# xandercai/JSPSR

Hardware: AMD Instinct MI355X
Metric: Mpixels/sec fwd+bwd, JSPSR x8 on 512^2 DEM tiles (higher is better)
Workload: dtype bf16; 1 GPU; jspsr_r8_img_msk (image+mask guided, 43.87M params), 8 x 512x512 tiles per GPU, train step (fwd + L1/L2/Sobel loss + bwd + grad all-reduce + AdamW); storage policy: bf16 activations / gradients / MFMA operands, fp32 accumulation, BatchNorm statistics, master weights and optimizer, and the generator head (affinity logits + offsets) kept as fp32 planes; tiles_per_gpu=8, tile=512, global_tiles=8, parallelism=dp1, step_mode=eager

## Files before the change

### include/jspsr_hip.h

```cpp
#ifndef JSPSR_HIP_H
#define JSPSR_HIP_H

#include <stddef.h>
#include <stdint.h>

#ifdef __cplusplus
extern "C" {
#endif

#define JSPSR_OK 0
#define JSPSR_EINVAL (-1)
#define JSPSR_EALIGN (-2)

typedef void* jspsr_stream_t;

int jspsr_abi_version(void);
long long jspsr_launch_count(const char* what);
int jspsr_conv_dynamic_queue(int on);
const char* jspsr_last_error(void);

int jspsr_prop_forward_f32(const float* dem, const float* weight, const float* offset,
                           int offset_channels, const float* wk, const float* b0, float scale,
                           float* out, int B, int H, int W, jspsr_stream_t stream);

size_t jspsr_prop_backward_workspace_bytes(int B, int H, int W);

int jspsr_prop_backward_f32(const float* grad_out, const float* dem, const float* weight,
                            const float* offset, int offset_channels, const float* wk,
                            float* grad_weight, float* grad_offset, float* grad_wk,
                            float* grad_b0, void* workspace, int B, int H, int W,
                            jspsr_stream_t stream);

int jspsr_prop_backward_fold_f32(const void* workspace, int B, int H, int W, float* grad_wk, float* grad_b0,
                                 jspsr_stream_t stream);

int jspsr_prop_step_forward_f32(const float* dem, const float* weight, const float* offset, int offset_channels,
                                const float* wk, const float* b0, float scale, int normalize, float* out,
                                int B, int H, int W, jspsr_stream_t stream);
size_t jspsr_prop_step_backward_workspace_bytes(int B, int H, int W);
int jspsr_prop_step_backward_f32(const float* grad_out, const float* dem, const float* weight, const float* offset,
                                 int offset_channels, const float* wk, float scale, int normalize, int accumulate,
                                 float* grad_weight, float* grad_offset, float* grad_dem, float* grad_wk,
                                 float* grad_b0, void* workspace, int B, int H, int W, jspsr_stream_t stream);

int jspsr_prop_head_forward(int dtype, const float* dem, const void* head, const float* wk, const float* b0,
                            float scale, float* out, int B, int H, int W, jspsr_stream_t stream);
size_t jspsr_prop_head_backward_workspace_bytes(int B, int H, int W);
int jspsr_prop_head_backward(int dtype, const float* grad_out, const float* dem, const void* head, const float* wk,
                             void* grad_head, float* grad_wk, float* grad_b0, void* workspace, int B, int H, int W,
                             jspsr_stream_t stream);

int jspsr_tiles_crop_f32(const float* x, float* out, int C, int H, int W, int k, int stride, int n_x, jspsr_stream_t stream);
int jspsr_tiles_merge_f32(const float* tiles, const float* ramp, float* out, int n_x, int k, int border_px, int stride,
                          jspsr_stream_t stream);
int jspsr_mirror_pad_f32(const float* x, float* out, int C, int H, int W, int n, jspsr_stream_t stream);
int jspsr_elev_scale_f32(const float* in, float* out, long long n, int descale, int elev_log, double elev_min, double elev_max,
                         double base_elev, jspsr_stream_t stream);

#define JSPSR_BATCH_LOG 1
#define JSPSR_BATCH_SCALE_MASK 2
#define JSPSR_BATCH_IMAGE_11 4
#define JSPSR_BATCH_LABEL_11 8
#define JSPSR_BATCH_IMAGE_255 16
#define JSPSR_BATCH_FLAGS 31
int jspsr_batch_make(const void* const* src, const long long* src_bytes, float* const* out, const int* channels,
                     const int* coff, const int* cpitch, const long long* scenes, int n_scenes, const int* samples, int B,
                     int k, int flags, double elev_min, double elev_max, int mask_div, jspsr_stream_t stream);

int jspsr_prop_logits_forward_f32(const float* dem, const float* head, const float* wk, const float* b0, float scale,
                                  float* out, int B, int H, int W, jspsr_stream_t stream);
int jspsr_prop_logits_backward_f32(const float* grad_out, const float* dem, const float* head, const float* wk,
                                   float* grad_head, float* grad_wk, float* grad_b0, void* workspace, int B, int H, int W,
                                   jspsr_stream_t stream);

int jspsr_head_ok(int dtype, int B, int H, int W, int Cin);
int jspsr_head_forward(int dtype, const void* x, int x_cstride, int x_coff, int Cin, const float* w25, const float* b25,
                       float* planes, int B, int H, int W, jspsr_stream_t stream);
size_t jspsr_head_backward_workspace_bytes(int B, int H, int W);
int jspsr_head_backward(int dtype, const float* grad_planes, const float* w25, int Cin, void* grad_x, int gx_cstride,
                        int gx_coff, void* grad_nhwc32, float* grad_b25, void* workspace, int B, int H, int W,
                        jspsr_stream_t stream);

int jspsr_conv_head1_forward(int dtype, const void* x, int x_cstride, int x_coff, int C, const float* w, const float* bias,
                             float* y, int B, int H, int W, jspsr_stream_t stream);
size_t jspsr_conv_head1_workspace_bytes(int B, int H, int W, int C);
int jspsr_conv_head1_backward(int dtype, const float* dy, const void* x, int x_cstride, int x_coff, int C, const float* w,
                              void* dx, int dx_cstride, int dx_coff, float* dw, float* db, void* workspace, int B, int H,
                              int W, jspsr_stream_t stream);

#define JSPSR_F32 0
#define JSPSR_BF16 1

int jspsr_pack_weight(int dtype, const float* w, void* packed, int O, int I, int KH, int KW,
                      int mode, int c_pad, jspsr_stream_t stream);

typedef struct jspsr_pack_desc {
  const float* w;
  void* out;
  long long start;
  long long total;
  int O, I, KH, KW;
  int mode;
  int c_pad;
  int dtype;
  int reserved;
} jspsr_pack_desc;
int jspsr_pack_chunk(void);
int jspsr_pack_weights_multi(const jspsr_pack_desc* descs, int n, long long total_blocks, jspsr_stream_t stream);

int jspsr_conv2d_stats_rows(int B, int OH, int OW);
int jspsr_conv2d_in_affine_ok(int dtype, int Cin, int KH, int KW, int stride);
int jspsr_conv2d_forward(int dtype, const void* in, const void* wpack, const float* bias, void* out,
                         int B, int IH, int IW, int Cin, int in_cstride, int in_coff, int Cout,
                         int out_cstride, int out_coff, int KH, int KW, int stride, int pad, int relu,
                         float* stats, const float* scale, const void* addend, int add_cstride,
                         const float* in_affine, int in_relu, jspsr_stream_t stream);

int jspsr_conv2d_dgrad_reduce_ok(int dtype, int B, int IH, int IW, int Cg, int Cin, int KH, int KW, int stride, int pad);
int jspsr_conv2d_dgrad(int dtype, const void* gout, const void* wpack_t, const float* bias, void* gin,
                       int B, int OH, int OW, int Cg, int g_cstride, int g_coff, int IH, int IW,
                       int Cin, int in_cstride, int in_coff, int KH, int KW, int stride, int pad,
                       int relu, const void* addend, int add_cstride, const float* scale,
                       const void* red_x, int red_cstride, const float* red_par, float* red_out, jspsr_stream_t stream);

size_t jspsr_conv2d_wgrad_workspace_bytes(int dtype, int B, int OH, int OW, int Cg, int Cx, int KH, int KW);
int jspsr_conv2d_wgrad_x_affine_ok(int dtype, int B, int OH, int OW, int Cg, int Cx, int KH, int KW, int stride, int pad);
int jspsr_conv2d_wgrad(int dtype, const void* G, int Cg, int g_cstride, int g_coff, const void* X, int Cx,
                       int x_cstride, int x_coff, float* dW, int R, int C, int B, int OH, int OW,
                       int IH, int IW, int KH, int KW, int stride, int pad, int accumulate,
                       const float* x_affine, int x_relu, void* workspace, jspsr_stream_t stream);

size_t jspsr_reduce_workspace_bytes(int dtype, int C, int nseg);

int jspsr_bn_forward(int dtype, const void* x, int x_cs, int x_coff, const void* res, int r_cs, int r_coff,
                     void* y, int y_cs, int y_coff, const float* gamma, const float* beta,
                     float* running_mean, float* running_var, float momentum, float eps, int training,
                     int relu, float res_scale, float* save_mean, float* save_invstd, long long npix, int C,
                     const float* ext_partial, int ext_rows, const float* res_affine, float* affine_out,
                     void* workspace, jspsr_stream_t stream);

int jspsr_bn_fold(const float* gamma, const float* beta, const float* running_mean, const float* running_var,
                  float eps, float res_scale, int C, float* scale, float* shift, jspsr_stream_t stream);

int jspsr_bn_reduce_params(const float* gamma, const float* beta, const float* save_mean, const float* save_invstd, int C,
                           float* par, jspsr_stream_t stream);
int jspsr_bn_backward(int dtype, const void* dy, int dy_cs, int dy_coff, const void* y, int y_cs, int y_coff,
                      const void* x, int x_cs, int x_coff, const float* gamma, const float* beta, const float* save_mean,
                      const float* save_invstd, int training, int relu, float res_scale, void* dx, void* dres,
                      float* dgamma, float* dbeta, int accumulate, long long npix, int C, void* workspace,
                      const float* ext_partial, int ext_rows, jspsr_stream_t stream);

int jspsr_act_backward(int dtype, const void* dy, int dy_cs, int dy_coff, const void* y, int y_cs, int relu, void* dz,
                       int dz_cs, float* dbias, long long npix, int C, void* workspace, jspsr_stream_t stream);

int jspsr_gate_pool(int dtype, const void* x, int B, long long npix, int C, float* avg, float* mx, int* amax,
                    void* workspace, jspsr_stream_t stream);
int jspsr_gate_scale(int dtype, const void* x, const float* s, void* y, int B, long long npix, int C,
                     jspsr_stream_t stream);
int jspsr_gate_backward_reduce(int dtype, const void* dy, const void* x, float* ds, int B, long long npix, int C,
                               void* workspace, jspsr_stream_t stream);
int jspsr_gate_backward_apply(int dtype, const void* dy, const float* s, const float* davg, const float* dmax,
                              const int* amax, void* dx, int B, long long npix, int C, jspsr_stream_t stream);

size_t jspsr_loss_workspace_bytes(int B, int H, int W);
int jspsr_loss_forward(const float* pred, const float* gt, float w1, float w2, float wg, float* losses,
                       void* workspace, int B, int H, int W, jspsr_stream_t stream);
int jspsr_loss_backward(const float* pred, const float* gt, const float* grad_total, float w1, float w2,
                        float wg, float* grad_pred, const void* workspace, int B, int H, int W,
                        jspsr_stream_t stream);

size_t jspsr_loss_menu_workspace_bytes(int terms, int planes, int H, int W);
int jspsr_loss_menu_forward(const float* pred, const float* gt, int terms, int planes, int H, int W, int n_keys,
                            const int* key_slot, const double* key_weight, const float* base_losses, float* out,
                            void* workspace, jspsr_stream_t stream);
int jspsr_loss_menu_backward(const float* pred, const float* gt, int terms, int planes, int H, int W,
                             const double* slot_weight, const float* grad_total, float* grad_pred,
                             const void* workspace, jspsr_stream_t stream);
size_t jspsr_ssim_workspace_bytes(int planes, int H, int W, int same);
int jspsr_ssim_forward(const float* pred, const float* gt, int planes, int H, int W, int same, const float* window11,
                       float* out, void* workspace, jspsr_stream_t stream);

size_t jspsr_metrics_workspace_bytes(int H, int W);
int jspsr_metrics_forward(const float* pred, const float* gt, int H, int W, float border, float value_min,
                          float value_max, int elev_log, float* scores, void* workspace, jspsr_stream_t stream);

size_t jspsr_scores_batch_workspace_bytes(int B, int H, int W);
int jspsr_scores_batch_forward(const float* pred, const float* gt, int B, int H, int W, float border, float value_min,
                               float value_max, int elev_log, float* scores, void* workspace, jspsr_stream_t stream);

int jspsr_adamw_step(float* param, const float* grad, float* exp_avg, float* exp_avg_sq, long long n, float lr,
                     float beta1, float beta2, float eps, float weight_decay, int step, jspsr_stream_t stream);
int jspsr_adamw_step_dev(float* param, const float* grad, float* exp_avg, float* exp_avg_sq, long long n,
                         const float* hyper, jspsr_stream_t stream);

#define JSPSR_OPT_SGD 0
#define JSPSR_OPT_ADAM 1
#define JSPSR_OPT_ADAMW 2
#define JSPSR_OPT_RMSPROP 3
size_t jspsr_optim_workspace_bytes(void);
int jspsr_optim_step(int kind, float* param, const float* grad, float* state1, float* state2, long long n, float lr, float a,
                     float b, float eps, float weight_decay, int step, const float* hyper, float* grad_range, void* workspace,
                     jspsr_stream_t stream);
size_t jspsr_tensor_ranges_workspace_bytes(void);
int jspsr_tensor_ranges(int count, const void* const* tensors, const long long* numel, const int* dtypes, float* table,
                        void* workspace, jspsr_stream_t stream);

int jspsr_gate_mlp_forward(const float* avg, const float* mx, const float* w1, const float* w2, int B, int C, int Ch,
                           float* s, float* hid, jspsr_stream_t stream);
size_t jspsr_gate_mlp_backward_workspace_bytes(int B, int C, int Ch);
int jspsr_gate_mlp_backward(const float* ds, const float* s, const float* hid, const float* avg, const float* mx,
                            const float* w1, const float* w2, int B, int C, int Ch, float* davg, float* dmax, float* dw1,
                            float* dw2, void* workspace, jspsr_stream_t stream);

int jspsr_nchw_to_nhwc(int dtype, const float* src, void* dst, int B, int C, int H, int W, int c_pad, jspsr_stream_t stream);

#ifdef __cplusplus
}
#endif
#endif
```

### jspsr_amd/_lib.py

```python
from __future__ import annotations

import ctypes
import os
import subprocess
import threading

_HERE = os.path.dirname(os.path.abspath(__file__))
SO_PATH = os.environ.get("JSPSR_LAB_LIB") or os.path.join(_HERE, "lib", "libjspsr_hip.so")
CSRC = os.path.join(_HERE, "csrc")
ABI_VERSION = 20

_lock = threading.Lock()
_lib = None

c_p = ctypes.c_void_p
c_i = ctypes.c_int
c_f = ctypes.c_float
c_ll = ctypes.c_longlong

SIGNATURES = {
    "jspsr_abi_version": (c_i, []),
    "jspsr_launch_count": (c_ll, [ctypes.c_char_p]),
    "jspsr_conv_dynamic_queue": (c_i, [c_i]),
    "jspsr_last_error": (ctypes.c_char_p, []),
    "jspsr_prop_forward_f32": (c_i, [c_p, c_p, c_p, c_i, c_p, c_p, c_f, c_p, c_i, c_i, c_i, c_p]),
    "jspsr_prop_backward_workspace_bytes": (ctypes.c_size_t, [c_i, c_i, c_i]),
    "jspsr_prop_backward_f32": (c_i, [c_p] * 4 + [c_i] + [c_p] * 6 + [c_i, c_i, c_i, c_p]),
    "jspsr_prop_backward_fold_f32": (c_i, [c_p, c_i, c_i, c_i, c_p, c_p, c_p]),
    "jspsr_prop_step_forward_f32": (c_i, [c_p, c_p, c_p, c_i, c_p, c_p, c_f, c_i, c_p, c_i, c_i, c_i, c_p]),
    "jspsr_prop_step_backward_workspace_bytes": (ctypes.c_size_t, [c_i, c_i, c_i]),
    "jspsr_prop_step_backward_f32": (c_i, [c_p] * 4 + [c_i, c_p, c_f, c_i, c_i] + [c_p] * 6 + [c_i, c_i, c_i, c_p]),
    "jspsr_prop_head_forward": (c_i, [c_i, c_p, c_p, c_p, c_p, c_f, c_p, c_i, c_i, c_i, c_p]),
    "jspsr_prop_head_backward_workspace_bytes": (ctypes.c_size_t, [c_i, c_i, c_i]),
    "jspsr_prop_head_backward": (c_i, [c_i] + [c_p] * 8 + [c_i, c_i, c_i, c_p]),
    "jspsr_prop_logits_forward_f32": (c_i, [c_p, c_p, c_p, c_p, c_f, c_p, c_i, c_i, c_i, c_p]),
    "jspsr_prop_logits_backward_f32": (c_i, [c_p] * 8 + [c_i, c_i, c_i, c_p]),
    "jspsr_head_ok": (c_i, [c_i] * 5),
    "jspsr_head_forward": (c_i, [c_i, c_p, c_i, c_i, c_i, c_p, c_p, c_p, c_i, c_i, c_i, c_p]),
    "jspsr_head_backward_workspace_bytes": (ctypes.c_size_t, [c_i, c_i, c_i]),
    "jspsr_head_backward": (c_i, [c_i, c_p, c_p, c_i, c_p, c_i, c_i, c_p, c_p, c_p, c_i, c_i, c_i, c_p]),
    "jspsr_conv_head1_forward": (c_i, [c_i, c_p, c_i, c_i, c_i, c_p, c_p, c_p, c_i, c_i, c_i, c_p]),
    "jspsr_conv_head1_workspace_bytes": (ctypes.c_size_t, [c_i, c_i, c_i, c_i]),
    "jspsr_conv_head1_backward": (c_i, [c_i, c_p, c_p, c_i, c_i, c_i, c_p, c_p, c_i, c_i, c_p, c_p, c_p, c_i, c_i, c_i, c_p]),
    "jspsr_pack_weight": (c_i, [c_i, c_p, c_p] + [c_i] * 6 + [c_p]),
    "jspsr_pack_chunk": (c_i, []),
    "jspsr_pack_weights_multi": (c_i, [c_p, c_i, c_ll, c_p]),
    "jspsr_conv2d_stats_rows": (c_i, [c_i, c_i, c_i]),
    "jspsr_conv2d_in_affine_ok": (c_i, [c_i] * 5),
    "jspsr_conv2d_forward": (c_i, [c_i] + [c_p] * 4 + [c_i] * 14 + [c_p, c_p, c_p, c_i, c_p, c_i, c_p]),
    "jspsr_bn_fold": (c_i, [c_p, c_p, c_p, c_p, c_f, c_f, c_i, c_p, c_p, c_p]),
    "jspsr_conv2d_dgrad_reduce_ok": (c_i, [c_i] * 10),
    "jspsr_conv2d_dgrad": (c_i, [c_i] + [c_p] * 4 + [c_i] * 16 + [c_p, c_i, c_p, c_p, c_i, c_p, c_p, c_p]),
    "jspsr_conv2d_wgrad_workspace_bytes": (ctypes.c_size_t, [c_i] * 8),
    "jspsr_conv2d_wgrad_x_affine_ok": (c_i, [c_i] * 10),
    "jspsr_conv2d_wgrad": (c_i, [c_i, c_p, c_i, c_i, c_i, c_p, c_i, c_i, c_i, c_p] + [c_i] * 12 + [c_p, c_i, c_p, c_p]),
    "jspsr_reduce_workspace_bytes": (ctypes.c_size_t, [c_i, c_i, c_i]),
    "jspsr_bn_forward": (c_i, [c_i, c_p, c_i, c_i, c_p, c_i, c_i, c_p, c_i, c_i, c_p, c_p, c_p, c_p, c_f, c_f, c_i,
                               c_i, c_f, c_p, c_p, c_ll, c_i, c_p, c_i, c_p, c_p, c_p, c_p]),
    "jspsr_bn_reduce_params": (c_i, [c_p, c_p, c_p, c_p, c_i, c_p, c_p]),
    "jspsr_bn_backward": (c_i, [c_i, c_p, c_i, c_i, c_p, c_i, c_i, c_p, c_i, c_i, c_p, c_p, c_p, c_p, c_i, c_i, c_f,
                                c_p, c_p, c_p, c_p, c_i, c_ll, c_i, c_p, c_p, c_i, c_p]),
    "jspsr_act_backward": (c_i, [c_i, c_p, c_i, c_i, c_p, c_i, c_i, c_p, c_i, c_p, c_ll, c_i, c_p, c_p]),
    "jspsr_gate_pool": (c_i, [c_i, c_p, c_i, c_ll, c_i, c_p, c_p, c_p, c_p, c_p]),
    "jspsr_gate_scale": (c_i, [c_i, c_p, c_p, c_p, c_i, c_ll, c_i, c_p]),
    "jspsr_gate_backward_reduce": (c_i, [c_i, c_p, c_p, c_p, c_i, c_ll, c_i, c_p, c_p]),
    "jspsr_gate_backward_apply": (c_i, [c_i, c_p, c_p, c_p, c_p, c_p, c_p, c_i, c_ll, c_i, c_p]),
    "jspsr_loss_workspace_bytes": (ctypes.c_size_t, [c_i, c_i, c_i]),
    "jspsr_loss_forward": (c_i, [c_p, c_p, c_f, c_f, c_f, c_p, c_p, c_i, c_i, c_i, c_p]),
    "jspsr_loss_backward": (c_i, [c_p, c_p, c_p, c_f, c_f, c_f, c_p, c_p, c_i, c_i, c_i, c_p]),
    "jspsr_loss_menu_workspace_bytes": (ctypes.c_size_t, [c_i, c_i, c_i, c_i]),
    "jspsr_loss_menu_forward": (c_i, [c_p, c_p, c_i, c_i, c_i, c_i, c_i, c_p, c_p, c_p, c_p, c_p, c_p]),
    "jspsr_loss_menu_backward": (c_i, [c_p, c_p, c_i, c_i, c_i, c_i, c_p, c_p, c_p, c_p, c_p]),
    "jspsr_ssim_workspace_bytes": (ctypes.c_size_t, [c_i, c_i, c_i, c_i]),
    "jspsr_ssim_forward": (c_i, [c_p, c_p, c_i, c_i, c_i, c_i, c_p, c_p, c_p, c_p]),
    "jspsr_metrics_workspace_bytes": (ctypes.c_size_t, [c_i, c_i]),
    "jspsr_metrics_forward": (c_i, [c_p, c_p, c_i, c_i, c_f, c_f, c_f, c_i, c_p, c_p, c_p]),
    "jspsr_scores_batch_workspace_bytes": (ctypes.c_size_t, [c_i, c_i, c_i]),
    "jspsr_scores_batch_forward": (c_i, [c_p, c_p, c_i, c_i, c_i, c_f, c_f, c_f, c_i, c_p, c_p, c_p]),
    "jspsr_adamw_step": (c_i, [c_p, c_p, c_p, c_p, c_ll, c_f, c_f, c_f, c_f, c_f, c_i, c_p]),
    "jspsr_adamw_step_dev": (c_i, [c_p, c_p, c_p, c_p, c_ll, c_p, c_p]),
    "jspsr_optim_workspace_bytes": (ctypes.c_size_t, []),
    "jspsr_optim_step": (c_i, [c_i, c_p, c_p, c_p, c_p, c_ll, c_f, c_f, c_f, c_f, c_f, c_i, c_p, c_p, c_p, c_p]),
    "jspsr_tensor_ranges_workspace_bytes": (ctypes.c_size_t, []),
    "jspsr_tensor_ranges": (c_i, [c_i, c_p, c_p, c_p, c_p, c_p, c_p]),
    "jspsr_tiles_crop_f32":(c_i, [c_p, c_p] + [c_i] * 6 + [c_p]),
    "jspsr_tiles_merge_f32": (c_i, [c_p, c_p, c_p, c_i, c_i, c_i, c_i, c_p]),
    "jspsr_mirror_pad_f32": (c_i, [c_p, c_p, c_i, c_i, c_i, c_i, c_p]),
    "jspsr_elev_scale_f32": (c_i, [c_p, c_p, c_ll, c_i, c_i, ctypes.c_double, ctypes.c_double, ctypes.c_double, c_p]),
    "jspsr_gate_mlp_forward": (c_i, [c_p, c_p, c_p, c_p, c_i, c_i, c_i, c_p, c_p, c_p]),
    "jspsr_gate_mlp_backward_workspace_bytes": (ctypes.c_size_t, [c_i, c_i, c_i]),
    "jspsr_gate_mlp_backward": (c_i, [c_p] * 7 + [c_i, c_i, c_i] + [c_p] * 6),
    "jspsr_batch_make": (c_i, [c_p] * 7 + [c_i, c_p, c_i, c_i, c_i, ctypes.c_double, ctypes.c_double, c_i, c_p]),
    "jspsr_nchw_to_nhwc": (c_i, [c_i, c_p, c_p, c_i, c_i, c_i, c_i, c_i, c_p]),
}


class JspsrHipError(RuntimeError):
    pass


def build(verbose: bool = False) -> str:
    cmd = ["make", "-C", CSRC, "-j4"] + ([] if verbose else ["-s"])
    subprocess.check_call(cmd)
    return SO_PATH


def load():
    global _lib
    if _lib is not None:
        return _lib
    with _lock:
        if _lib is not None:
            return _lib
        if not os.path.exists(SO_PATH):
            raise JspsrHipError(
                f"{SO_PATH} is missing: build it with `python -c 'import __graft_entry__ as g; g.build()'` "
                "(hipcc --offload-arch=gfx950). jspsr_amd has no fallback path."
            )
        import torch
        lib = ctypes.CDLL(SO_PATH)
        for name, (res, args) in SIGNATURES.items():
            fn = getattr(lib, name)
            fn.restype = res
            fn.argtypes = args
        v = lib.jspsr_abi_version()
        if v != ABI_VERSION:
            raise JspsrHipError(f"libjspsr_hip.so ABI {v} != binding ABI {ABI_VERSION}: rebuild")
        _lib = lib
    return _lib


calls = 0


def check(code: int, what: str):
    global calls
    calls += 1
    if code != 0:
        msg = load().jspsr_last_error().decode(errors="replace")
        raise JspsrHipError(f"{what} failed (code {code}): {msg}")
```

### jspsr_amd/csrc/common.hip

```cpp
#include "common.h"

#include <atomic>
#include <cstring>

namespace jspsr {

namespace {
struct Slot {
  std::atomic<const char*> name{nullptr};
  std::atomic<long long> n{0};
};
Slot g_slots[128];

void count_launch(const char* what) {
  for (Slot& s : g_slots) {
    const char* cur = s.name.load(std::memory_order_acquire);
    if (cur == nullptr) {
      const char* expect = nullptr;
      if (s.name.compare_exchange_strong(expect, what, std::memory_order_acq_rel)) cur = what; else cur = expect;
    }
    if (cur == what) { s.n.fetch_add(1, std::memory_order_relaxed); return; }
  }
}
}

char* err_buf() {
  static thread_local char buf[512] = {0};
  return buf;
}

int fail(int code, const char* fmt, ...) {
  va_list ap;
  va_start(ap, fmt);
  vsnprintf(err_buf(), 512, fmt, ap);
  va_end(ap);
  return code;
}

int check_launch(const char* what) {
  count_launch(what);
  hipError_t e = hipGetLastError();
  if (e != hipSuccess) return fail(static_cast<int>(e), "%s: %s", what, hipGetErrorString(e));
  return JSPSR_OK;
}

}

namespace jspsr {
std::atomic<int> g_conv_dynq{-1};
int conv_dynq_override() { return g_conv_dynq.load(std::memory_order_relaxed); }
}

extern "C" int jspsr_abi_version(void) { return 20; }
extern "C" int jspsr_conv_dynamic_queue(int on) { return jspsr::g_conv_dynq.exchange(on < 0 ? -1 : (on ? 1 : 0), std::memory_order_relaxed); }
extern "C" long long jspsr_launch_count(const char* what) {
  if (!what) return -1;
  long long n = 0;
  for (jspsr::Slot& s : jspsr::g_slots) {
    const char* cur = s.name.load(std::memory_order_acquire);
    if (cur && strcmp(cur, what) == 0) n += s.n.load(std::memory_order_relaxed);
  }
  return n;
}
extern "C" const char* jspsr_last_error(void) { return jspsr::err_buf(); }
```

### jspsr_amd/csrc/elementwise.hip

```cpp
#include "common.h"

#include <cstdlib>

namespace {

using namespace jspsr;

constexpr int TX = 64, TY = 4;

template <typename T> struct V;
template <> struct V<float> { static constexpr int N = 4; };
template <> struct V<__bf16> { static constexpr int N = 8; };

template <typename T, int N>
struct Pack { T v[N]; };

template <typename T>
__device__ __forceinline__ uint4 load_raw(const T* p) { return *reinterpret_cast<const uint4*>(p); }
template <typename T>
__device__ __forceinline__ void unpack(const uint4& raw, float (&f)[V<T>::N]) {
  if constexpr (sizeof(T) == 4) {
    f[0] = __uint_as_float(raw.x); f[1] = __uint_as_float(raw.y); f[2] = __uint_as_float(raw.z); f[3] = __uint_as_float(raw.w);
  } else {
    const unsigned w[4] = {raw.x, raw.y, raw.z, raw.w};
#pragma unroll
    for (int i = 0; i < 4; ++i) {
      f[2 * i] = __uint_as_float(w[i] << 16);
      f[2 * i + 1] = __uint_as_float(w[i] & 0xffff0000u);
    }
  }
}

__device__ __forceinline__ unsigned bf16_bits(float x) {
  const __bf16 h = (__bf16)x;
  return (unsigned)__builtin_bit_cast(unsigned short, h);
}

template <typename T>
__device__ __forceinline__ void store_vec(T* p, const float (&f)[V<T>::N]) {
  uint4 raw;
  if constexpr (sizeof(T) == 4) {
    raw.x = __float_as_uint(f[0]); raw.y = __float_as_uint(f[1]); raw.z = __float_as_uint(f[2]); raw.w = __float_as_uint(f[3]);
  } else {
    raw.x = bf16_bits(f[0]) | (bf16_bits(f[1]) << 16);
    raw.y = bf16_bits(f[2]) | (bf16_bits(f[3]) << 16);
    raw.z = bf16_bits(f[4]) | (bf16_bits(f[5]) << 16);
    raw.w = bf16_bits(f[6]) | (bf16_bits(f[7]) << 16);
  }
  *reinterpret_cast<uint4*>(p) = raw;
}

struct Slice {
  const void* p;
  int cs, coff;
};

struct RedGeom {
  long long npix;
  int nseg;
  int C;
  int chunks;
  long long chunk_pix;
  int lpp;
  int pl;
};

struct LaneMap {
  int c;
  int sub;
};
template <int N>
__device__ __forceinline__ LaneMap lane_map(const RedGeom& g) {
  LaneMap m;
  const int tx = threadIdx.x;
  m.sub = tx / g.lpp;
  const int cg = blockIdx.y * TX + (tx - m.sub * g.lpp);
  m.c = (m.sub < g.pl) ? cg * N : g.C;
  return m;
}

RedGeom make_red(long long npix, int nseg, int C, int vec) {
  RedGeom g;
  g.npix = npix; g.nseg = nseg; g.C = C;
  const int gy = (C / vec + TX - 1) / TX;
  static const int target = [] { const char* e = getenv("JSPSR_RED_BLOCKS"); return e ? atoi(e) : 1024; }();
  long long want = target / ((long long)gy * nseg);
  if (want < 1) want = 1;
  long long chunks = (npix + 63) / 64;
  if (chunks > want) chunks = want;
  if (chunks < 1) chunks = 1;
  g.chunk_pix = (npix + chunks - 1) / chunks;
  g.chunks = (int)((npix + g.chunk_pix - 1) / g.chunk_pix);
  const int groups = C / vec;
  g.lpp = groups < TX ? groups : TX;
  g.pl = TX / g.lpp;
  return g;
}
dim3 red_grid(const RedGeom& g, int vec) { return dim3(g.nseg * g.chunks, (g.C / vec + TX - 1) / TX); }

#ifndef K4_PIX_FLY
#define K4_PIX_FLY 4
#endif
constexpr int PIX_FLY = K4_PIX_FLY;
template <typename T, int K, int NTEN, typename L, typename F>
__device__ __forceinline__ void reduce_pixels_mlp(const RedGeom& g, float* __restrict__ partial, L&& load, F&& use) {
  constexpr int N = V<T>::N;
  __shared__ float red[TY][K][TX * N];
  const int tx = threadIdx.x, ty = threadIdx.y;
  const LaneMap lm = lane_map<N>(g);
  const int c = lm.c;
  const int seg = blockIdx.x / g.chunks, chunk = blockIdx.x % g.chunks;
  float acc[K][N];
#pragma unroll
  for (int k = 0; k < K; ++k)
#pragma unroll
    for (int i = 0; i < N; ++i) acc[k][i] = 0.f;
  const long long p0 = chunk * g.chunk_pix;
  const long long p1 = (p0 + g.chunk_pix < g.npix) ? p0 + g.chunk_pix : g.npix;
  if (c < g.C) {
    const long long step = TY * g.pl, base = (long long)seg * g.npix;
    long long p = p0 + ty * g.pl + lm.sub;
    for (; p + (PIX_FLY - 1) * step < p1; p += PIX_FLY * step) {
      uint4 raw[PIX_FLY][NTEN];
#pragma unroll
      for (int u = 0; u < PIX_FLY; ++u) load(base + p + u * step, c, raw[u]);
#pragma unroll
      for (int u = 0; u < PIX_FLY; ++u) use(base + p + u * step, c, raw[u], acc);
    }
    for (; p < p1; p += step) {
      uint4 raw[NTEN];
      load(base + p, c, raw);
      use(base + p, c, raw, acc);
    }
  }
#pragma unroll
  for (int k = 0; k < K; ++k)
#pragma unroll
    for (int i = 0; i < N; ++i) red[ty][k][tx * N + i] = acc[k][i];
  __syncthreads();
  if (ty == 0 && lm.sub == 0 && c < g.C) {
    float* dst = partial + ((size_t)blockIdx.x * K) * g.C + c;
#pragma unroll
    for (int k = 0; k < K; ++k)
#pragma unroll
      for (int i = 0; i < N; ++i) {
        float s = 0.f;
        for (int j = 0; j < g.pl; ++j)
#pragma unroll
          for (int y = 0; y < TY; ++y) s += red[y][k][(tx + j * g.lpp) * N + i];
        dst[(size_t)k * g.C + i] = s;
      }
  }
}
template <typename T, int NTEN, typename L, typename F>
__device__ __forceinline__ void for_pixels_mlp(const RedGeom& g, L&& load, F&& use) {
  constexpr int N = V<T>::N;
  const LaneMap lm = lane_map<N>(g);
  const int c = lm.c;
  if (c >= g.C) return;
  const int seg = blockIdx.x / g.chunks, chunk = blockIdx.x % g.chunks;
  const long long p0 = chunk * g.chunk_pix;
  const long long p1 = (p0 + g.chunk_pix < g.npix) ? p0 + g.chunk_pix : g.npix;
  const long long step = TY * g.pl, base = (long long)seg * g.npix;
  long long p = p0 + threadIdx.y * g.pl + lm.sub;
  for (; p + (PIX_FLY - 1) * step < p1; p += PIX_FLY * step) {
    uint4 raw[PIX_FLY][NTEN];
#pragma unroll
    for (int u = 0; u < PIX_FLY; ++u) load(base + p + u * step, c, raw[u]);
#pragma unroll
    for (int u = 0; u < PIX_FLY; ++u) use(p + u * step, base + p + u * step, c, raw[u]);
  }
  for (; p < p1; p += step) {
    uint4 raw[NTEN];
    load(base + p, c, raw);
    use(p, base + p, c, raw);
  }
}

template <int N>
__device__ __forceinline__ void load_param(const float* __restrict__ p, float (&f)[N]) {
#pragma unroll
  for (int i = 0; i < N; i += 4) {
    const float4 v = *reinterpret_cast<const float4*>(p + i);
    f[i] = v.x; f[i + 1] = v.y; f[i + 2] = v.z; f[i + 3] = v.w;
  }
}

__device__ __forceinline__ double wave_sum_rows(const float* __restrict__ partial, int rows, size_t pitch, size_t off) {
  const int lane = threadIdx.x & 63;
  double s = 0.0;
  for (int r = lane; r < rows; r += 64) s += (double)partial[(size_t)r * pitch + off];
#pragma unroll
  for (int d = 32; d > 0; d >>= 1) s += __shfl_xor(s, d, 64);
  return s;
}

__device__ __forceinline__ void wave_sum_rows2(const float* __restrict__ partial, int rows, size_t pitch, size_t off0, size_t off1,
                                               double& s0, double& s1) {
  const int lane = threadIdx.x & 63;
  double a = 0.0, b = 0.0;
  int r = lane;
  for (; r + 192 < rows; r += 256) {
    const float x0 = partial[(size_t)r * pitch + off0], x1 = partial[(size_t)(r + 64) * pitch + off0];
    const float x2 = partial[(size_t)(r + 128) * pitch + off0], x3 = partial[(size_t)(r + 192) * pitch + off0];
    const float y0 = partial[(size_t)r * pitch + off1], y1 = partial[(size_t)(r + 64) * pitch + off1];
    const float y2 = partial[(size_t)(r + 128) * pitch + off1], y3 = partial[(size_t)(r + 192) * pitch + off1];
    a += (double)x0; a += (double)x1; a += (double)x2; a += (double)x3;
    b += (double)y0; b += (double)y1; b += (double)y2; b += (double)y3;
  }
  for (; r < rows; r += 64) {
    a += (double)partial[(size_t)r * pitch + off0];
    b += (double)partial[(size_t)r * pitch + off1];
  }
#pragma unroll
  for (int d = 32; d > 0; d >>= 1) {
    a += __shfl_xor(a, d, 64);
    b += __shfl_xor(b, d, 64);
  }
  s0 = a;
  s1 = b;
}

template <typename T>
__global__ __launch_bounds__(TX * TY) void bn_stats_kernel(const T* __restrict__ x, int cs, int coff, RedGeom g,
                                                          float* __restrict__ partial) {
  constexpr int N = V<T>::N;
  reduce_pixels_mlp<T, 2, 1>(
      g, partial, [&](long long pix, int c, uint4 (&raw)[1]) { raw[0] = load_raw<T>(x + (size_t)pix * cs + coff + c); },
      [&](long long, int, const uint4 (&raw)[1], float (&acc)[2][N]) {
        float f[N];
        unpack<T>(raw[0], f);
#pragma unroll
        for (int i = 0; i < N; ++i) { acc[0][i] += f[i]; acc[1][i] += f[i] * f[i]; }
      });
}

__global__ void fold_rows_kernel(const float* __restrict__ in, int nin, int width, int nout, float* __restrict__ out) {
  const int r = blockIdx.x, j = blockIdx.y * blockDim.x + threadIdx.x;
  if (j >= width) return;
  float s = 0.f;
  int i = r;
  for (; i + 7 * nout < nin; i += 8 * nout) {
    float v[8];
#pragma unroll
    for (int k = 0; k < 8; ++k) v[k] = in[(size_t)(i + k * nout) * width + j];
#pragma unroll
    for (int k = 0; k < 8; ++k) s += v[k];
  }
  for (; i < nin; i += nout) s += in[(size_t)i * width + j];
  out[(size_t)r * width + j] = s;
}

__global__ void bn_finalize_kernel(const float* __restrict__ partial, int rows, int C, long long count,
                                   const float* __restrict__ gamma, const float* __restrict__ beta,
                                   float* __restrict__ running_mean, float* __restrict__ running_var,
                                   float momentum, float eps, int training, float* __restrict__ save_mean,
                                   float* __restrict__ save_invstd, float* __restrict__ scale,
                                   float* __restrict__ shift) {
  const int c = blockIdx.x * (blockDim.x >> 6) + (threadIdx.x >> 6);
  if (c >= C) return;
  float mean, var;
  double s = 0.0, ss = 0.0;
  if (training) {
    wave_sum_rows2(partial, rows, (size_t)2 * C, c, (size_t)C + c, s, ss);
  }
  if ((threadIdx.x & 63) != 0) return;
  if (training) {
    const double m = s / (double)count;
    double v = ss / (double)count - m * m;
    if (v < 0.0) v = 0.0;
    mean = (float)m;
    var = (float)v;
    if (running_mean) {
      const double unb = count > 1 ? v * (double)count / (double)(count - 1) : v;
      running_mean[c] = (1.f - momentum) * running_mean[c] + momentum * mean;
      running_var[c] = (1.f - momentum) * running_var[c] + momentum * (float)unb;
    }
  } else {
    mean = running_mean[c];
    var = running_var[c];
  }
  const float invstd = 1.0f / sqrtf(var + eps);
  save_mean[c] = mean;
  save_invstd[c] = invstd;
  const float sc = gamma[c] * invstd;
  scale[c] = sc;
  shift[c] = beta[c] - mean * sc;
}

__global__ void bn_fold_kernel(const float* __restrict__ gamma, const float* __restrict__ beta,
                               const float* __restrict__ mean, const float* __restrict__ var, float eps, float res_scale,
                               int C, float* __restrict__ scale, float* __restrict__ shift) {
  const int c = blockIdx.x * blockDim.x + threadIdx.x;
  if (c >= C) return;
  const float sc = gamma[c] * (1.0f / sqrtf(var[c] + eps));
  scale[c] = sc * res_scale;
  shift[c] = (beta[c] - mean[c] * sc) * res_scale;
}

template <typename T, bool RES>
__global__ __launch_bounds__(TX * TY) void bn_apply_kernel(const T* __restrict__ x, int x_cs, int x_coff,
                                                          const T* __restrict__ res, int r_cs, int r_coff,
                                                          T* __restrict__ y, int y_cs, int y_coff,
                                                          const float* __restrict__ scale, const float* __restrict__ shift,
                                                          const float* __restrict__ raff, float res_scale, int relu, RedGeom g) {
  constexpr int N = V<T>::N;
  float sc[N], sh[N], rsc[N], rsh[N];
  const int c0 = lane_map<N>(g).c;
  if (c0 < g.C) { load_param<N>(scale + c0, sc); load_param<N>(shift + c0, sh); }
  if (raff && c0 < g.C) { load_param<N>(raff + c0, rsc); load_param<N>(raff + g.C + c0, rsh); }
  constexpr int NTEN = RES ? 2 : 1;
  for_pixels_mlp<T, NTEN>(
      g,
      [&](long long pix, int c, uint4 (&raw)[NTEN]) {
        raw[0] = load_raw<T>(x + (size_t)pix * x_cs + x_coff + c);
        if constexpr (RES) raw[1] = load_raw<T>(res + (size_t)pix * r_cs + r_coff + c);
      },
      [&](long long, long long pix, int c, const uint4 (&raw)[NTEN]) {
        float f[N], r[N];
        unpack<T>(raw[0], f);
        if constexpr (RES) unpack<T>(raw[1], r);
#pragma unroll
        for (int k = 0; k < N; ++k) {
          float v = f[k] * sc[k] + sh[k];
          if (RES) v = v * res_scale + (raff ? r[k] * rsc[k] + rsh[k] : r[k]);
          if (relu) v = fmaxf(v, 0.f);
          f[k] = v;
        }
        store_vec<T>(y + (size_t)pix * y_cs + y_coff + c, f);
      });
}

template <typename T, int RELU>
__global__ __launch_bounds__(TX * TY) void bn_bwd_reduce_kernel(const T* __restrict__ dy, int dy_cs, int dy_coff,
                                                               const T* __restrict__ y, int y_cs, int y_coff,
                                                               const T* __restrict__ x, int x_cs, int x_coff,
                                                               const float* __restrict__ mean,
                                                               const float* __restrict__ invstd,
                                                               const float* __restrict__ gamma,
                                                               const float* __restrict__ beta, RedGeom g,
                                                               float* __restrict__ partial) {
  constexpr int N = V<T>::N, NTEN = RELU == 1 ? 3 : 2;
  float mu[N], is[N], ga[N], be[N];
  const int c0 = lane_map<N>(g).c;
  if (c0 < g.C) {
    load_param<N>(mean + c0, mu); load_param<N>(invstd + c0, is);
    if (RELU == 2) { load_param<N>(gamma + c0, ga); load_param<N>(beta + c0, be); }
  }
  reduce_pixels_mlp<T, 2, NTEN>(
      g, partial,
      [&](long long pix, int c, uint4 (&raw)[NTEN]) {
        raw[0] = load_raw<T>(dy + (size_t)pix * dy_cs + dy_coff + c);
        raw[1] = load_raw<T>(x + (size_t)pix * x_cs + x_coff + c);
        if constexpr (RELU == 1) raw[2] = load_raw<T>(y + (size_t)pix * y_cs + y_coff + c);
      },
      [&](long long, int, const uint4 (&raw)[NTEN], float (&acc)[2][N]) {
        float d[N], xv[N], yv[N];
        unpack<T>(raw[0], d);
        unpack<T>(raw[1], xv);
        if constexpr (RELU == 1) unpack<T>(raw[2], yv);
#pragma unroll
        for (int i = 0; i < N; ++i) {
          const float xhat = (xv[i] - mu[i]) * is[i];
          const bool off = RELU == 1 ? !(yv[i] > 0.f) : (RELU == 2 ? !(ga[i] * xhat + be[i] > 0.f) : false);
          const float dz = off ? 0.f : d[i];
          acc[0][i] += dz;
          acc[1][i] += dz * xhat;
        }
      });
}

__global__ void bn_bwd_finalize_kernel(const float* __restrict__ partial, int rows, int C, long long count,
                                       const float* __restrict__ gamma, const float* __restrict__ invstd,
                                       int training, float res_scale, int accumulate, float* __restrict__ dgamma,
                                       float* __restrict__ dbeta, float* __restrict__ coef) {
  const int c = blockIdx.x * (blockDim.x >> 6) + (threadIdx.x >> 6);
  if (c >= C) return;
  double s, sx;
  wave_sum_rows2(partial, rows, (size_t)2 * C, c, (size_t)C + c, s, sx);
  if ((threadIdx.x & 63) != 0) return;
  dbeta[c] = (accumulate ? dbeta[c] : 0.f) + (float)(s * res_scale);
  dgamma[c] = (accumulate ? dgamma[c] : 0.f) + (float)(sx * res_scale);
  const float k = gamma[c] * invstd[c] * res_scale;
  coef[c] = k;
  coef[C + c] = training ? (float)(s / (double)count) : 0.f;
  coef[2 * C + c] = training ? (float)(sx / (double)count) : 0.f;
}

template <typename T, int RELU>
__global__ __launch_bounds__(TX * TY) void bn_bwd_apply_kernel(const T* __restrict__ dy, int dy_cs, int dy_coff,
                                                              const T* __restrict__ y, int y_cs, int y_coff,
                                                              const T* __restrict__ x, int x_cs, int x_coff,
                                                              const float* __restrict__ mean, const float* __restrict__ invstd,
                                                              const float* __restrict__ gamma, const float* __restrict__ beta,
                                                              const float* __restrict__ coef,
                                                              T* __restrict__ dx, T* __restrict__ dres, RedGeom g) {
  constexpr int N = V<T>::N, NTEN = RELU == 1 ? 3 : 2;
  const int C = g.C;
  float mu[N], is[N], k0[N], ka[N], kb[N], ga[N], be[N];
  const int c0 = lane_map<N>(g).c;
  if (c0 < C) {
    load_param<N>(mean + c0, mu); load_param<N>(invstd + c0, is);
    load_param<N>(coef + c0, k0); load_param<N>(coef + C + c0, ka); load_param<N>(coef + 2 * C + c0, kb);
    if (RELU == 2) { load_param<N>(gamma + c0, ga); load_param<N>(beta + c0, be); }
  }
  for_pixels_mlp<T, NTEN>(
      g,
      [&](long long pix, int c, uint4 (&raw)[NTEN]) {
        raw[0] = load_raw<T>(dy + (size_t)pix * dy_cs + dy_coff + c);
        raw[1] = load_raw<T>(x + (size_t)pix * x_cs + x_coff + c);
        if constexpr (RELU == 1) raw[2] = load_raw<T>(y + (size_t)pix * y_cs + y_coff + c);
      },
      [&](long long, long long pix, int c, const uint4 (&raw)[NTEN]) {
        float d[N], xv[N], yv[N], o[N];
        unpack<T>(raw[0], d);
        unpack<T>(raw[1], xv);
        if constexpr (RELU == 1) unpack<T>(raw[2], yv);
#pragma unroll
        for (int k = 0; k < N; ++k) {
          const float xhat = (xv[k] - mu[k]) * is[k];
          const bool off = RELU == 1 ? !(yv[k] > 0.f) : (RELU == 2 ? !(ga[k] * xhat + be[k] > 0.f) : false);
          const float dz = off ? 0.f : d[k];
          d[k] = dz;
          o[k] = k0[k] * (dz - ka[k] - xhat * kb[k]);
        }
        store_vec<T>(dx + (size_t)pix * C + c, o);
        if (dres) store_vec<T>(dres + (size_t)pix * C + c, d);
      });
}

template <typename T, bool RELU>
__global__ __launch_bounds__(TX * TY) void act_bwd_kernel(const T* __restrict__ dy, int dy_cs, int dy_coff,
                                                         const T* __restrict__ y, int y_cs, int relu,
                                                         T* __restrict__ dz, int dz_cs, RedGeom g,
                                                         float* __restrict__ partial) {
  constexpr int N = V<T>::N;
  constexpr int NTEN = RELU ? 2 : 1;
  (void)relu;
  reduce_pixels_mlp<T, 1, NTEN>(
      g, partial,
      [&](long long pix, int c, uint4 (&raw)[NTEN]) {
        raw[0] = load_raw<T>(dy + (size_t)pix * dy_cs + dy_coff + c);
        if constexpr (RELU) raw[1] = load_raw<T>(y + (size_t)pix * y_cs + c);
      },
      [&](long long pix, int c, const uint4 (&raw)[NTEN], float (&acc)[1][N]) {
        float d[N], yv[N];
        unpack<T>(raw[0], d);
        if constexpr (RELU) unpack<T>(raw[1], yv);
#pragma unroll
        for (int i = 0; i < N; ++i) {
          if (RELU && !(yv[i] > 0.f)) d[i] = 0.f;
          acc[0][i] += d[i];
        }
        if (dz) store_vec<T>(dz + (size_t)pix * dz_cs + c, d);
      });
}

__global__ void sum_rows_kernel(const float* __restrict__ partial, int rows, int K, int k, int C, float* __restrict__ out) {
  const int c = blockIdx.x * (blockDim.x >> 6) + (threadIdx.x >> 6);
  if (c >= C) return;
  const double s = wave_sum_rows(partial, rows, (size_t)K * C, (size_t)k * C + c);
  if ((threadIdx.x & 63) == 0) out[c] = (float)s;
}

template <typename T>
__global__ __launch_bounds__(TX * TY) void gate_pool_kernel(const T* __restrict__ x, RedGeom g,
                                                           float* __restrict__ psum, float* __restrict__ pmax,
                                                           int* __restrict__ pidx) {
  constexpr int N = V<T>::N;
  __shared__ float rs[TY][TX * N], rm[TY][TX * N];
  __shared__ int ri[TY][TX * N];
  const int tx = threadIdx.x, ty = threadIdx.y;
  const LaneMap lm = lane_map<N>(g);
  const int c = lm.c;
  const int seg = blockIdx.x / g.chunks, chunk = blockIdx.x % g.chunks;
  float s[N], m[N];
  int idx[N];
#pragma unroll
  for (int i = 0; i < N; ++i) { s[i] = 0.f; m[i] = -INFINITY; idx[i] = 0x7fffffff; }
  const long long p0 = chunk * g.chunk_pix;
  const long long p1 = (p0 + g.chunk_pix < g.npix) ? p0 + g.chunk_pix : g.npix;
  if (c < g.C) {
    const long long step = TY * g.pl;
    long long p = p0 + ty * g.pl + lm.sub;
    auto take = [&](const uint4& raw, long long pp) {
      float f[N];
      unpack<T>(raw, f);
#pragma unroll
      for (int i = 0; i < N; ++i) {
        s[i] += f[i];
        if (f[i] > m[i]) { m[i] = f[i]; idx[i] = (int)pp; }
      }
    };
    for (; p + (PIX_FLY - 1) * step < p1; p += PIX_FLY * step) {
      uint4 raw[PIX_FLY];
#pragma unroll
      for (int u = 0; u < PIX_FLY; ++u) raw[u] = load_raw<T>(x + ((size_t)seg * g.npix + p + u * step) * g.C + c);
#pragma unroll
      for (int u = 0; u < PIX_FLY; ++u) take(raw[u], p + u * step);
    }
    for (; p < p1; p += step) take(load_raw<T>(x + ((size_t)seg * g.npix + p) * g.C + c), p);
  }
#pragma unroll
  for (int i = 0; i < N; ++i) { rs[ty][tx * N + i] = s[i]; rm[ty][tx * N + i] = m[i]; ri[ty][tx * N + i] = idx[i]; }
  __syncthreads();
  if (ty == 0 && lm.sub == 0 && c < g.C) {
#pragma unroll
    for (int i = 0; i < N; ++i) {
      float ss = 0.f, mm = -INFINITY;
      int ii = 0x7fffffff;
      for (int q = 0; q < g.pl; ++q)
#pragma unroll
      for (int y = 0; y < TY; ++y) {
        const int col = (tx + q * g.lpp) * N + i;
        ss += rs[y][col];
        const float v = rm[y][col];
        const int j = ri[y][col];
        if (v > mm || (v == mm && j < ii)) { mm = v; ii = j; }
      }
      const size_t o = (size_t)blockIdx.x * g.C + c + i;
      psum[o] = ss; pmax[o] = mm; pidx[o] = ii;
    }
  }
}

__global__ void gate_pool_finalize_kernel(const float* __restrict__ psum, const float* __restrict__ pmax,
                                          const int* __restrict__ pidx, int chunks, int C, long long npix,
                                          float* __restrict__ avg, float* __restrict__ mx, int* __restrict__ amax) {
  const int c = blockIdx.x * blockDim.x + threadIdx.x, b = blockIdx.y;
  if (c >= C) return;
  double s = 0.0;
  float m = -INFINITY;
  int ii = 0x7fffffff;
  int r = 0;
  for (; r + 8 <= chunks; r += 8) {
    float ps[8], pm[8];
    int pi[8];
#pragma unroll
    for (int k = 0; k < 8; ++k) {
      const size_t o = ((size_t)b * chunks + r + k) * C + c;
      ps[k] = psum[o]; pm[k] = pmax[o]; pi[k] = pidx[o];
    }
#pragma unroll
    for (int k = 0; k < 8; ++k) {
      s += (double)ps[k];
      if (pm[k] > m || (pm[k] == m && pi[k] < ii)) { m = pm[k]; ii = pi[k]; }
    }
  }
  for (; r < chunks; ++r) {
    const size_t o = ((size_t)b * chunks + r) * C + c;
    s += (double)psum[o];
    if (pmax[o] > m || (pmax[o] == m && pidx[o] < ii)) { m = pmax[o]; ii = pidx[o]; }
  }
  avg[(size_t)b * C + c] = (float)(s / (double)npix);
  mx[(size_t)b * C + c] = m;
  amax[(size_t)b * C + c] = ii;
}

template <typename T>
__global__ __launch_bounds__(TX * TY) void gate_scale_kernel(const T* __restrict__ x, const float* __restrict__ s,
                                                            T* __restrict__ y, RedGeom g) {
  constexpr int N = V<T>::N;
  float sv[N];
  const int c0 = lane_map<N>(g).c;
  if (c0 < g.C) load_param<N>(s + (size_t)(blockIdx.x / g.chunks) * g.C + c0, sv);
  for_pixels_mlp<T, 1>(
      g, [&](long long pix, int c, uint4 (&raw)[1]) { raw[0] = load_raw<T>(x + (size_t)pix * g.C + c); },
      [&](long long, long long pix, int c, const uint4 (&raw)[1]) {
        float f[N];
        unpack<T>(raw[0], f);
#pragma unroll
        for (int k = 0; k < N; ++k) f[k] *= sv[k];
        store_vec<T>(y + (size_t)pix * g.C + c, f);
      });
}

template <typename T>
__global__ __launch_bounds__(TX * TY) void gate_bwd_reduce_kernel(const T* __restrict__ dy, const T* __restrict__ x,
                                                                 RedGeom g, float* __restrict__ partial) {
  constexpr int N = V<T>::N;
  reduce_pixels_mlp<T, 1, 2>(
      g, partial,
      [&](long long pix, int c, uint4 (&raw)[2]) {
        raw[0] = load_raw<T>(dy + (size_t)pix * g.C + c);
        raw[1] = load_raw<T>(x + (size_t)pix * g.C + c);
      },
      [&](long long, int, const uint4 (&raw)[2], float (&acc)[1][N]) {
        float d[N], xv[N];
        unpack<T>(raw[0], d);
        unpack<T>(raw[1], xv);
#pragma unroll
        for (int i = 0; i < N; ++i) acc[0][i] += d[i] * xv[i];
      });
}

__global__ void gate_bwd_finalize_kernel(const float* __restrict__ partial, int chunks, int C, float* __restrict__ ds) {
  const int c = blockIdx.x * blockDim.x + threadIdx.x, b = blockIdx.y;
  if (c >= C) return;
  double s = 0.0;
  int r = 0;
  for (; r + 8 <= chunks; r += 8) {
    float v[8];
#pragma unroll
    for (int k = 0; k < 8; ++k) v[k] = partial[((size_t)b * chunks + r + k) * C + c];
#pragma unroll
    for (int k = 0; k < 8; ++k) s += (double)v[k];
  }
  for (; r < chunks; ++r) s += (double)partial[((size_t)b * chunks + r) * C + c];
  ds[(size_t)b * C + c] = (float)s;
}

template <typename T>
__global__ __launch_bounds__(TX * TY) void gate_bwd_apply_kernel(const T* __restrict__ dy, const float* __restrict__ s,
                                                                const float* __restrict__ davg, const float* __restrict__ dmax,
                                                                const int* __restrict__ amax, T* __restrict__ dx, RedGeom g) {
  constexpr int N = V<T>::N;
  float sv[N], da[N], dm[N];
  int am[N];
  const int c0 = lane_map<N>(g).c;
  const float inv = 1.f / (float)g.npix;
  if (c0 < g.C) {
    const size_t o = (size_t)(blockIdx.x / g.chunks) * g.C + c0;
    load_param<N>(s + o, sv); load_param<N>(davg + o, da); load_param<N>(dmax + o, dm);
#pragma unroll
    for (int k = 0; k < N; ++k) { am[k] = amax[o + k]; da[k] *= inv; }
  }
  for_pixels_mlp<T, 1>(
      g, [&](long long pix, int c, uint4 (&raw)[1]) { raw[0] = load_raw<T>(dy + (size_t)pix * g.C + c); },
      [&](long long p, long long pix, int c, const uint4 (&raw)[1]) {
        float f[N];
        unpack<T>(raw[0], f);
#pragma unroll
        for (int k = 0; k < N; ++k) f[k] = f[k] * sv[k] + da[k] + (am[k] == (int)p ? dm[k] : 0.f);
        store_vec<T>(dx + (size_t)pix * g.C + c, f);
      });
}

int ew_blocks(long long total) {
  long long b = (total + 255) / 256;
  return (int)(b < 1 ? 1 : (b > 4096 ? 4096 : b));
}

int check_c(int dtype, int C, const char* what) {
  if (dtype != JSPSR_F32 && dtype != JSPSR_BF16) return fail(JSPSR_EINVAL, "%s: bad dtype", what);
  const int vec = dtype == JSPSR_F32 ? 4 : 8;
  if (C <= 0 || C % vec) return fail(JSPSR_EINVAL, "%s: C=%d must be a multiple of %d", what, C, vec);
  return JSPSR_OK;
}

}

#define DISPATCH(dtype, CALL)                    \
  do {                                           \
    if ((dtype) == JSPSR_F32) { using T = float; CALL; } else { using T = __bf16; CALL; } \
  } while (0)

extern "C" size_t jspsr_reduce_workspace_bytes(int dtype, int C, int nseg) {
  if (C <= 0 || nseg <= 0) return 0;
  const int vec = dtype == JSPSR_F32 ? 4 : 8;
  const RedGeom g = make_red(1LL << 40, nseg, C, vec);
  const size_t rows = (size_t)nseg * g.chunks;
  return (rows * 3 + 4) * (size_t)C * sizeof(float) + 64;
}

extern "C" int jspsr_bn_forward(int dtype, const void* x, int x_cs, int x_coff, const void* res, int r_cs, int r_coff,
                                void* y, int y_cs, int y_coff, const float* gamma, const float* beta,
                                float* running_mean, float* running_var, float momentum, float eps, int training,
                                int relu, float res_scale, float* save_mean, float* save_invstd, long long npix, int C,
                                const float* ext_partial, int ext_rows, const float* res_affine, float* affine_out,
                                void* workspace, jspsr_stream_t stream) {
  if (int e = check_c(dtype, C, "bn_forward")) return e;
  if (!x || (!y && !affine_out) || !gamma || !beta || !save_mean || !save_invstd || !workspace || npix <= 0)
    return fail(JSPSR_EINVAL, "bn_forward: null pointer or empty tensor");
  if (res_affine && !res) return fail(JSPSR_EINVAL, "bn_forward: res_affine without a residual operand");
  if (!training && (!running_mean || !running_var)) return fail(JSPSR_EINVAL, "bn_forward: eval mode needs running stats");
  const int vec = dtype == JSPSR_F32 ? 4 : 8;
  if (x_cs % vec || x_coff % vec || y_cs % vec || y_coff % vec || (res && (r_cs % vec || r_coff % vec)))
    return fail(JSPSR_EINVAL, "bn_forward: channel pitches/offsets must be multiples of %d", vec);
  hipStream_t s = static_cast<hipStream_t>(stream);
  float* ws = static_cast<float*>(workspace);
  float* scale = affine_out ? affine_out : ws;
  float* shift = affine_out ? affine_out + C : ws + C;
  float* partial = ws + 2 * C;
  int rows = 0;
  if (training && ext_partial) {
    if (ext_rows <= 0) return fail(JSPSR_EINVAL, "bn_forward: ext_rows must be positive");
    rows = ext_rows < 256 ? ext_rows : 256;
    if (ext_rows > 256) {
      hipLaunchKernelGGL(fold_rows_kernel, dim3(rows, (2 * C + 255) / 256), dim3(256), 0, s, ext_partial, ext_rows, 2 * C, rows, partial);
      if (int e = check_launch("bn_fold_rows")) return e;
    } else {
      (void)hipMemcpyAsync(partial, ext_partial, (size_t)ext_rows * 2 * C * sizeof(float), hipMemcpyDeviceToDevice, s);
    }
  } else if (training) {
    const RedGeom g = make_red(npix, 1, C, vec);
    rows = g.chunks;
    DISPATCH(dtype, hipLaunchKernelGGL(bn_stats_kernel<T>, red_grid(g, vec), dim3(TX, TY), 0, s,
                                       static_cast<const T*>(x), x_cs, x_coff, g, partial));
    if (int e = check_launch("bn_stats")) return e;
  }
  hipLaunchKernelGGL(bn_finalize_kernel, dim3((C + 3) / 4), dim3(256), 0, s, partial, rows, C, npix, gamma, beta,
                     running_mean, running_var, momentum, eps, training, save_mean, save_invstd, scale, shift);
  if (int e = check_launch("bn_finalize")) return e;
  if (!y) return JSPSR_OK;
  const RedGeom ga = make_red(npix, 1, C, vec);
#define BN_APPLY(R) DISPATCH(dtype, hipLaunchKernelGGL((bn_apply_kernel<T, R>), red_grid(ga, vec), dim3(TX, TY), 0, s,             \
                                     static_cast<const T*>(x), x_cs, x_coff, static_cast<const T*>(res), r_cs, r_coff,        \
                                     static_cast<T*>(y), y_cs, y_coff, scale, shift, res_affine, res_scale, relu, ga))
  if (res) { BN_APPLY(true); } else { BN_APPLY(false); }
#undef BN_APPLY
  return check_launch("bn_apply");
}

__global__ void bn_reduce_params_kernel(const float* __restrict__ gamma, const float* __restrict__ beta, const float* __restrict__ mean,
                                        const float* __restrict__ invstd, int C, float* __restrict__ par) {
  const int c = blockIdx.x * blockDim.x + threadIdx.x;
  if (c >= C) return;
  const float a = gamma[c] * invstd[c];
  par[c] = a;
  par[C + c] = beta[c] - a * mean[c];
  par[2 * C + c] = invstd[c];
  par[3 * C + c] = -mean[c] * invstd[c];
}

extern "C" int jspsr_bn_reduce_params(const float* gamma, const float* beta, const float* save_mean, const float* save_invstd, int C,
                                      float* par, jspsr_stream_t stream) {
  if (!gamma || !beta || !save_mean || !save_invstd || !par || C <= 0) return fail(JSPSR_EINVAL, "bn_reduce_params: bad arguments");
  hipLaunchKernelGGL(bn_reduce_params_kernel, dim3((C + 255) / 256), dim3(256), 0, static_cast<hipStream_t>(stream), gamma, beta,
                     save_mean, save_invstd, C, par);
  return check_launch("bn_reduce_params");
}

extern "C" int jspsr_bn_backward(int dtype, const void* dy, int dy_cs, int dy_coff, const void* y, int y_cs, int y_coff,
                                 const void* x, int x_cs, int x_coff, const float* gamma, const float* beta, const float* save_mean,
                                 const float* save_invstd, int training, int relu, float res_scale, void* dx, void* dres,
                                 float* dgamma, float* dbeta, int accumulate, long long npix, int C, void* workspace,
                                 const float* ext_partial, int ext_rows, jspsr_stream_t stream) {
  if (int e = check_c(dtype, C, "bn_backward")) return e;
  if (!dy || !x || !gamma || !save_mean || !save_invstd || !dx || !dgamma || !dbeta || !workspace || npix <= 0 ||
      (relu == 1 && !y) || (relu == 2 && !beta) || relu < 0 || relu > 2)
    return fail(JSPSR_EINVAL, "bn_backward: null pointer, empty tensor or bad relu mode");
  const int vec = dtype == JSPSR_F32 ? 4 : 8;
  if (dy_cs % vec || dy_coff % vec || x_cs % vec || x_coff % vec || (relu == 1 && (y_cs % vec || y_coff % vec)))
    return fail(JSPSR_EINVAL, "bn_backward: channel pitches/offsets must be multiples of %d", vec);
  hipStream_t s = static_cast<hipStream_t>(stream);
  float* ws = static_cast<float*>(workspace);
  float* coef = ws;
  float* partial = ws + 3 * C;
  const RedGeom g = make_red(npix, 1, C, vec);
#define BN_BWD_REDUCE(R) DISPATCH(dtype, hipLaunchKernelGGL((bn_bwd_reduce_kernel<T, R>), red_grid(g, vec), dim3(TX, TY), 0, s, \
                                     static_cast<const T*>(dy), dy_cs, dy_coff, static_cast<const T*>(y), y_cs, y_coff,     \
                                     static_cast<const T*>(x), x_cs, x_coff, save_mean, save_invstd, gamma, beta, g, partial))
  int rows = g.chunks;
  if (ext_partial) {
    if (ext_rows <= 0) return fail(JSPSR_EINVAL, "bn_backward: ext_rows must be positive");
    if (ext_rows > 1024) {
      rows = g.chunks < 1024 ? (g.chunks > 0 ? g.chunks : 1) : 1024;
      hipLaunchKernelGGL(fold_rows_kernel, dim3(rows, (2 * C + 255) / 256), dim3(256), 0, s, ext_partial, ext_rows, 2 * C, rows, partial);
      if (int e = check_launch("bn_fold_rows")) return e;
    } else {
      partial = const_cast<float*>(ext_partial);
      rows = ext_rows;
    }
  } else {
    if (relu == 0) { BN_BWD_REDUCE(0); } else if (relu == 1) { BN_BWD_REDUCE(1); } else { BN_BWD_REDUCE(2); }
    if (int e = check_launch("bn_bwd_reduce")) return e;
  }
#undef BN_BWD_REDUCE
  hipLaunchKernelGGL(bn_bwd_finalize_kernel, dim3((C + 3) / 4), dim3(256), 0, s, partial, rows, C, npix, gamma,
                     save_invstd, training, res_scale, accumulate, dgamma, dbeta, coef);
  if (int e = check_launch("bn_bwd_finalize")) return e;
#define BN_BWD_APPLY(R) DISPATCH(dtype, hipLaunchKernelGGL((bn_bwd_apply_kernel<T, R>), red_grid(g, vec), dim3(TX, TY), 0, s,  \
                                     static_cast<const T*>(dy), dy_cs, dy_coff, static_cast<const T*>(y), y_cs, y_coff,     \
                                     static_cast<const T*>(x), x_cs, x_coff, save_mean, save_invstd, gamma, beta, coef,     \
                                     static_cast<T*>(dx), static_cast<T*>(dres), g))
  if (relu == 0) { BN_BWD_APPLY(0); } else if (relu == 1) { BN_BWD_APPLY(1); } else { BN_BWD_APPLY(2); }
#undef BN_BWD_APPLY
  return check_launch("bn_bwd_apply");
}

extern "C" int jspsr_bn_fold(const float* gamma, const float* beta, const float* running_mean, const float* running_var,
                             float eps, float res_scale, int C, float* scale, float* shift, jspsr_stream_t stream) {
  if (!gamma || !beta || !running_mean || !running_var || !scale || !shift || C <= 0)
    return fail(JSPSR_EINVAL, "bn_fold: bad arguments");
  hipLaunchKernelGGL(bn_fold_kernel, dim3((C + 255) / 256), dim3(256), 0, static_cast<hipStream_t>(stream), gamma, beta,
                     running_mean, running_var, eps, res_scale, C, scale, shift);
  return check_launch("bn_fold");
}

extern "C" int jspsr_act_backward(int dtype, const void* dy, int dy_cs, int dy_coff, const void* y, int y_cs, int relu,
                                  void* dz, int dz_cs, float* dbias, long long npix, int C, void* workspace,
                                  jspsr_stream_t stream) {
  if (int e = check_c(dtype, C, "act_backward")) return e;
  if (!dy || (relu && !y) || !workspace || npix <= 0) return fail(JSPSR_EINVAL, "act_backward: null pointer or empty tensor");
  const int vec = dtype == JSPSR_F32 ? 4 : 8;
  if (dy_cs % vec || dy_coff % vec || (dz && dz_cs % vec) || (relu && (y_cs % vec || y_cs < C)))
    return fail(JSPSR_EINVAL, "act_backward: bad pitch");
  hipStream_t s = static_cast<hipStream_t>(stream);
  float* partial = static_cast<float*>(workspace);
  const RedGeom g = make_red(npix, 1, C, vec);
#define ACT_BWD(R) DISPATCH(dtype, hipLaunchKernelGGL((act_bwd_kernel<T, R>), red_grid(g, vec), dim3(TX, TY), 0, s, static_cast<const T*>(dy), \
                                     dy_cs, dy_coff, static_cast<const T*>(y), y_cs, relu, static_cast<T*>(dz), dz_cs, g, partial))
  if (relu) { ACT_BWD(true); } else { ACT_BWD(false); }
#undef ACT_BWD
  if (int e = check_launch("act_backward")) return e;
  if (dbias) {
    hipLaunchKernelGGL(sum_rows_kernel, dim3((C + 3) / 4), dim3(256), 0, s, partial, g.chunks, 1, 0, C, dbias);
    return check_launch("act_backward_bias");
  }
  return JSPSR_OK;
}

extern "C" int jspsr_gate_pool(int dtype, const void* x, int B, long long npix, int C, float* avg, float* mx, int* amax,
                               void* workspace, jspsr_stream_t stream) {
  if (int e = check_c(dtype, C, "gate_pool")) return e;
  if (!x || !avg || !mx || !amax || !workspace || B <= 0 || npix <= 0 || npix > 0x7fffffffLL)
    return fail(JSPSR_EINVAL, "gate_pool: bad arguments");
  const int vec = dtype == JSPSR_F32 ? 4 : 8;
  hipStream_t s = static_cast<hipStream_t>(stream);
  const RedGeom g = make_red(npix, B, C, vec);
  const size_t rows = (size_t)B * g.chunks;
  float* psum = static_cast<float*>(workspace);
  float* pmax = psum + rows * C;
  int* pidx = reinterpret_cast<int*>(pmax + rows * C);
  DISPATCH(dtype, hipLaunchKernelGGL(gate_pool_kernel<T>, red_grid(g, vec), dim3(TX, TY), 0, s, static_cast<const T*>(x), g,
                                     psum, pmax, pidx));
  if (int e = check_launch("gate_pool")) return e;
  hipLaunchKernelGGL(gate_pool_finalize_kernel, dim3((C + 255) / 256, B), dim3(256), 0, s, psum, pmax, pidx, g.chunks, C,
                     npix, avg, mx, amax);
  return check_launch("gate_pool_finalize");
}

extern "C" int jspsr_gate_scale(int dtype, const void* x, const float* s_, void* y, int B, long long npix, int C,
                                jspsr_stream_t stream) {
  if (int e = check_c(dtype, C, "gate_scale")) return e;
  if (!x || !s_ || !y || B <= 0 || npix <= 0) return fail(JSPSR_EINVAL, "gate_scale: bad arguments");
  const int vec = dtype == JSPSR_F32 ? 4 : 8;
  hipStream_t s = static_cast<hipStream_t>(stream);
  const RedGeom g = make_red(npix, B, C, vec);
  DISPATCH(dtype, hipLaunchKernelGGL(gate_scale_kernel<T>, red_grid(g, vec), dim3(TX, TY), 0, s,
                                     static_cast<const T*>(x), s_, static_cast<T*>(y), g));
  return check_launch("gate_scale");
}

extern "C" int jspsr_gate_backward_reduce(int dtype, const void* dy, const void* x, float* ds, int B, long long npix, int C,
                                          void* workspace, jspsr_stream_t stream) {
  if (int e = check_c(dtype, C, "gate_backward_reduce")) return e;
  if (!dy || !x || !ds || !workspace || B <= 0 || npix <= 0) return fail(JSPSR_EINVAL, "gate_backward_reduce: bad arguments");
  const int vec = dtype == JSPSR_F32 ? 4 : 8;
  hipStream_t s = static_cast<hipStream_t>(stream);
  const RedGeom g = make_red(npix, B, C, vec);
  float* partial = static_cast<float*>(workspace);
  DISPATCH(dtype, hipLaunchKernelGGL(gate_bwd_reduce_kernel<T>, red_grid(g, vec), dim3(TX, TY), 0, s,
                                     static_cast<const T*>(dy), static_cast<const T*>(x), g, partial));
  if (int e = check_launch("gate_backward_reduce")) return e;
  hipLaunchKernelGGL(gate_bwd_finalize_kernel, dim3((C + 255) / 256, B), dim3(256), 0, s, partial, g.chunks, C, ds);
  return check_launch("gate_backward_finalize");
}

extern "C" int jspsr_gate_backward_apply(int dtype, const void* dy, const float* s_, const float* davg, const float* dmax,
                                         const int* amax, void* dx, int B, long long npix, int C, jspsr_stream_t stream) {
  if (int e = check_c(dtype, C, "gate_backward_apply")) return e;
  if (!dy || !s_ || !davg || !dmax || !amax || !dx || B <= 0 || npix <= 0)
    return fail(JSPSR_EINVAL, "gate_backward_apply: bad arguments");
  const int vec = dtype == JSPSR_F32 ? 4 : 8;
  hipStream_t s = static_cast<hipStream_t>(stream);
  const RedGeom g = make_red(npix, B, C, vec);
  DISPATCH(dtype, hipLaunchKernelGGL(gate_bwd_apply_kernel<T>, red_grid(g, vec), dim3(TX, TY), 0, s,
                                     static_cast<const T*>(dy), s_, davg, dmax, amax, static_cast<T*>(dx), g));
  return check_launch("gate_backward_apply");
}

template <typename T>
__global__ __launch_bounds__(256) void nchw_to_nhwc_kernel(const float* __restrict__ src, T* __restrict__ dst, int C, long long HW,
                                                          long long npix, int Cpad) {
  constexpr int N = V<T>::N;
  for (long long p = blockIdx.x * 256LL + threadIdx.x; p < npix; p += (long long)gridDim.x * 256) {
    const long long b = p / HW, q = p - b * HW;
    const float* s = src + (size_t)b * C * HW + q;
    T* d = dst + (size_t)p * Cpad;
    for (int c0 = 0; c0 < Cpad; c0 += N) {
      float f[N];
#pragma unroll
      for (int i = 0; i < N; ++i) f[i] = c0 + i < C ? s[(size_t)(c0 + i) * HW] : 0.f;
      store_vec<T>(d + c0, f);
    }
  }
}

extern "C" int jspsr_nchw_to_nhwc(int dtype, const float* src, void* dst, int B, int C, int H, int W, int c_pad,
                                  jspsr_stream_t stream) {
  if (dtype != JSPSR_F32 && dtype != JSPSR_BF16) return fail(JSPSR_EINVAL, "nchw_to_nhwc: dtype must be JSPSR_F32 or JSPSR_BF16");
  const int vec = dtype == JSPSR_F32 ? 4 : 8;
  if (!src || !dst || B <= 0 || C <= 0 || H <= 0 || W <= 0 || c_pad < C || c_pad % vec)
    return fail(JSPSR_EINVAL, "nchw_to_nhwc: bad arguments (c_pad must be a multiple of %d and >= C)", vec);
  if (!aligned4(src) || !aligned16(dst)) return fail(JSPSR_EALIGN, "nchw_to_nhwc: src must be 4-byte, dst 16-byte aligned");
  const long long HW = (long long)H * W, npix = HW * B;
  const long long want = (npix + 255) / 256;
  const int blocks = (int)(want > 8192 ? 8192 : want);
  hipStream_t s = static_cast<hipStream_t>(stream);
  DISPATCH(dtype, hipLaunchKernelGGL(nchw_to_nhwc_kernel<T>, dim3(blocks), dim3(256), 0, s, src, static_cast<T*>(dst), C, HW, npix, c_pad));
  return check_launch("nchw_to_nhwc");
}

constexpr int GM_T = 256;

__global__ __launch_bounds__(GM_T) void gate_mlp_fwd_kernel(const float* __restrict__ avg, const float* __restrict__ mx,
                                                           const float* __restrict__ w1, const float* __restrict__ w2, int C, int Ch,
                                                           float* __restrict__ s, float* __restrict__ hid) {
  extern __shared__ float gm_lds[];
  const int b = blockIdx.x, tid = threadIdx.x, wave = tid >> 6, lane = tid & 63;
  const float* a = avg + (size_t)b * C;
  const float* m = mx + (size_t)b * C;
  for (int j = wave; j < Ch; j += GM_T / 64) {
    const float* w = w1 + (size_t)j * C;
    float da = 0.f, dm = 0.f;
    for (int c = lane; c < C; c += 64) { const float wv = w[c]; da += wv * a[c]; dm += wv * m[c]; }
#pragma unroll
    for (int d = 32; d > 0; d >>= 1) { da += __shfl_xor(da, d, 64); dm += __shfl_xor(dm, d, 64); }
    if (lane == 0) {
      const float ha = fmaxf(da, 0.f), hm = fmaxf(dm, 0.f);
      hid[((size_t)b * 2 + 0) * Ch + j] = ha;
      hid[((size_t)b * 2 + 1) * Ch + j] = hm;
      gm_lds[j] = ha + hm;
    }
  }
  __syncthreads();
  for (int c = tid; c < C; c += GM_T) {
    const float* w = w2 + (size_t)c * Ch;
    float z = 0.f;
    for (int j = 0; j < Ch; ++j) z += w[j] * gm_lds[j];
    s[(size_t)b * C + c] = 1.f / (1.f + expf(-z));
  }
}

__global__ __launch_bounds__(GM_T) void gate_mlp_bwd_kernel(const float* __restrict__ ds, const float* __restrict__ s,
                                                           const float* __restrict__ hid, const float* __restrict__ w1,
                                                           const float* __restrict__ w2, int C, int Ch, float* __restrict__ davg,
                                                           float* __restrict__ dmax, float* __restrict__ dzs, float* __restrict__ dhs) {
  extern __shared__ float gm_lds[];
  float* dz = gm_lds;
  float* dh = gm_lds + C;
  const int b = blockIdx.x, tid = threadIdx.x, wave = tid >> 6, lane = tid & 63;
  for (int c = tid; c < C; c += GM_T) {
    const float sv = s[(size_t)b * C + c], v = ds[(size_t)b * C + c] * sv * (1.f - sv);
    dz[c] = v;
    dzs[(size_t)b * C + c] = v;
  }
  __syncthreads();
  for (int j = wave; j < Ch; j += GM_T / 64) {
    float acc = 0.f;
    for (int c = lane; c < C; c += 64) acc += w2[(size_t)c * Ch + j] * dz[c];
#pragma unroll
    for (int d = 32; d > 0; d >>= 1) acc += __shfl_xor(acc, d, 64);
    if (lane == 0) {
      const float da = hid[((size_t)b * 2 + 0) * Ch + j] > 0.f ? acc : 0.f, dm = hid[((size_t)b * 2 + 1) * Ch + j] > 0.f ? acc : 0.f;
      dh[j] = da; dh[Ch + j] = dm;
      dhs[((size_t)b * 2 + 0) * Ch + j] = da;
      dhs[((size_t)b * 2 + 1) * Ch + j] = dm;
    }
  }
  __syncthreads();
  for (int c = tid; c < C; c += GM_T) {
    float ga = 0.f, gm = 0.f;
    for (int j = 0; j < Ch; ++j) { const float wv = w1[(size_t)j * C + c]; ga += wv * dh[j]; gm += wv * dh[Ch + j]; }
    davg[(size_t)b * C + c] = ga;
    dmax[(size_t)b * C + c] = gm;
  }
}

__global__ __launch_bounds__(GM_T) void gate_mlp_wgrad_kernel(const float* __restrict__ dzs, const float* __restrict__ dhs,
                                                             const float* __restrict__ hid, const float* __restrict__ avg,
                                                             const float* __restrict__ mx, int B, int C, int Ch,
                                                             float* __restrict__ dw1, float* __restrict__ dw2) {
  const long long n = (long long)C * Ch;
  for (long long i = blockIdx.x * (long long)GM_T + threadIdx.x; i < 2 * n; i += (long long)gridDim.x * GM_T) {
    if (i < n) {
      const int j = (int)(i / C), c = (int)(i - (long long)j * C);
      float g = 0.f;
      for (int b = 0; b < B; ++b)
        g += dhs[((size_t)b * 2 + 0) * Ch + j] * avg[(size_t)b * C + c] + dhs[((size_t)b * 2 + 1) * Ch + j] * mx[(size_t)b * C + c];
      dw1[i] = g;
    } else {
      const long long k = i - n;
      const int c = (int)(k / Ch), j = (int)(k - (long long)c * Ch);
      float g = 0.f;
      for (int b = 0; b < B; ++b) g += dzs[(size_t)b * C + c] * (hid[((size_t)b * 2 + 0) * Ch + j] + hid[((size_t)b * 2 + 1) * Ch + j]);
      dw2[k] = g;
    }
  }
}

extern "C" int jspsr_gate_mlp_forward(const float* avg, const float* mx, const float* w1, const float* w2, int B, int C, int Ch,
                                      float* s, float* hid, jspsr_stream_t stream) {
  if (!avg || !mx || !w1 || !w2 || !s || !hid || B <= 0 || C <= 0 || Ch <= 0 || Ch > 4096)
    return fail(JSPSR_EINVAL, "gate_mlp_forward: bad arguments");
  hipLaunchKernelGGL(gate_mlp_fwd_kernel, dim3(B), dim3(GM_T), Ch * sizeof(float), static_cast<hipStream_t>(stream), avg, mx, w1, w2,
                     C, Ch, s, hid);
  return check_launch("gate_mlp_forward");
}

extern "C" size_t jspsr_gate_mlp_backward_workspace_bytes(int B, int C, int Ch) {
  if (B <= 0 || C <= 0 || Ch <= 0) return 0;
  return ((size_t)B * C + (size_t)B * 2 * Ch) * sizeof(float);
}

extern "C" int jspsr_gate_mlp_backward(const float* ds, const float* s, const float* hid, const float* avg, const float* mx,
                                       const float* w1, const float* w2, int B, int C, int Ch, float* davg, float* dmax,
                                       float* dw1, float* dw2, void* workspace, jspsr_stream_t stream) {
  if (!ds || !s || !hid || !avg || !mx || !w1 || !w2 || !davg || !dmax || !dw1 || !dw2 || !workspace || B <= 0 || C <= 0 ||
      Ch <= 0 || (size_t)(C + 2 * Ch) * sizeof(float) > 64 * 1024)
    return fail(JSPSR_EINVAL, "gate_mlp_backward: bad arguments");
  float* dzs = static_cast<float*>(workspace);
  float* dhs = dzs + (size_t)B * C;
  hipStream_t st = static_cast<hipStream_t>(stream);
  hipLaunchKernelGGL(gate_mlp_bwd_kernel, dim3(B), dim3(GM_T), (C + 2 * Ch) * sizeof(float), st, ds, s, hid, w1, w2, C, Ch, davg, dmax,
                     dzs, dhs);
  if (int e = check_launch("gate_mlp_backward")) return e;
  const long long n2 = 2LL * C * Ch;
  const int blocks = (int)((n2 + GM_T - 1) / GM_T > 2048 ? 2048 : (n2 + GM_T - 1) / GM_T);
  hipLaunchKernelGGL(gate_mlp_wgrad_kernel, dim3(blocks), dim3(GM_T), 0, st, dzs, dhs, hid, avg, mx, B, C, Ch, dw1, dw2);
  return check_launch("gate_mlp_wgrad");
}
```

### jspsr_amd/kernels.py

```python
from __future__ import annotations

import torch

from . import _lib

F32, BF16 = 0, 1


def _dt(t: torch.Tensor) -> int:
    if t.dtype == torch.float32:
        return F32
    if t.dtype == torch.bfloat16:
        return BF16
    raise TypeError(f"unsupported dtype {t.dtype}")


def epc(dtype: torch.dtype) -> int:
    return 4 if dtype == torch.float32 else 8


def _stream() -> int:
    return torch.cuda.current_stream().cuda_stream


def _chk(t: torch.Tensor, name: str):
    if not t.is_cuda:
        raise RuntimeError(f"{name}: jspsr_amd kernels run on the GPU only (no CPU fallback)")
    if not t.is_contiguous():
        raise ValueError(f"{name}: expected a contiguous tensor")


def is_slice(t: torch.Tensor) -> bool:
    if t.dim() != 4 or t.stride(3) != 1:
        return False
    B, H, W, C = t.shape
    p = t.stride(2)
    if p < C or (H > 1 and t.stride(1) != W * p) or (B > 1 and t.stride(0) != H * W * p) or W == 1:
        return False
    return t.data_ptr() % 16 == 0 and (p * t.element_size()) % 16 == 0


def pitch(t: torch.Tensor) -> int:
    return t.shape[3] if t.is_contiguous() else t.stride(2)


def nhwc(t: torch.Tensor) -> torch.Tensor:
    return t if (t.is_contiguous() or is_slice(t)) else t.contiguous()


def _chk_s(t: torch.Tensor, name: str):
    if not t.is_cuda:
        raise RuntimeError(f"{name}: jspsr_amd kernels run on the GPU only (no CPU fallback)")
    if not (t.is_contiguous() or is_slice(t)):
        raise ValueError(f"{name}: expected a dense NHWC tensor or a channel slice of one")


def pack_weight(w: torch.Tensor, mode: int, c_pad: int, dtype: torch.dtype) -> torch.Tensor:
    _chk(w, "pack_weight")
    O, I, KH, KW = w.shape
    n = O if mode == 0 else I
    out = torch.empty((n, KH, KW, c_pad), dtype=dtype, device=w.device)
    lib = _lib.load()
    _lib.check(lib.jspsr_pack_weight(_dt(out), w.data_ptr(), out.data_ptr(), O, I, KH, KW, mode, c_pad, _stream()),
               "jspsr_pack_weight")
    return out


def fused_input_ok(dtype, B, OH, OW, Cin, Cout, KH, KW, stride, pad) -> bool:
    lib = _lib.load()
    dt = F32 if dtype == torch.float32 else BF16
    return bool(lib.jspsr_conv2d_in_affine_ok(dt, Cin, KH, KW, stride)) and \
        bool(lib.jspsr_conv2d_wgrad_x_affine_ok(dt, B, OH, OW, Cout, Cin, KH, KW, stride, pad))


def conv2d_forward(x, wpack, bias, stride, pad, relu=False, out=None, out_coff=0, cin=None, in_coff=0, stats=False,
                   scale=None, addend=None, in_affine=None, in_relu=False):
    _chk_s(x, "conv2d_forward")
    B, IH, IW, _ = x.shape
    Cs = pitch(x)
    Cout, KH, KW, Cin = wpack.shape
    if cin is not None and cin != Cin:
        raise ValueError("conv2d_forward: cin mismatch")
    OH = (IH + 2 * pad - KH) // stride + 1
    OW = (IW + 2 * pad - KW) // stride + 1
    if out is None:
        out = torch.empty((B, OH, OW, Cout), dtype=x.dtype, device=x.device)
    lib = _lib.load()
    st = None
    if stats:
        st = torch.empty((lib.jspsr_conv2d_stats_rows(B, OH, OW), 2, Cout), dtype=torch.float32, device=x.device)
    if addend is not None:
        _chk_s(addend, "conv2d_forward addend")
        if tuple(addend.shape) != (B, OH, OW, Cout) or addend.dtype != x.dtype:
            raise ValueError(f"conv2d_forward: addend {tuple(addend.shape)} {addend.dtype} does not match the result")
    _lib.check(lib.jspsr_conv2d_forward(_dt(x), x.data_ptr(), wpack.data_ptr(),
                                        bias.data_ptr() if bias is not None else None, out.data_ptr(),
                                        B, IH, IW, Cin, Cs, in_coff, Cout, pitch(out), out_coff,
                                        KH, KW, stride, pad, int(relu), st.data_ptr() if st is not None else None,
                                        scale.data_ptr() if scale is not None else None,
                                        addend.data_ptr() if addend is not None else None,
                                        pitch(addend) if addend is not None else 0,
                                        in_affine.data_ptr() if in_affine is not None else None, int(in_relu),
                                        _stream()), "jspsr_conv2d_forward")
    return (out, st) if stats else out


def dgrad_reduce_ok(dtype, B, IH, IW, Cg, Cin, KH, KW, stride, pad) -> bool:
    dt = F32 if dtype == torch.float32 else BF16
    return bool(_lib.load().jspsr_conv2d_dgrad_reduce_ok(dt, B, IH, IW, Cg, Cin, KH, KW, stride, pad))


def bn_reduce_params(gamma, beta, mean, invstd):
    C = gamma.numel()
    par = torch.empty((4, C), dtype=torch.float32, device=gamma.device)
    _lib.check(_lib.load().jspsr_bn_reduce_params(gamma.data_ptr(), beta.data_ptr(), mean.data_ptr(), invstd.data_ptr(), C,
                                                  par.data_ptr(), _stream()), "jspsr_bn_reduce_params")
    return par


def conv2d_dgrad(g, wpack_t, in_hw, stride, pad, bias=None, relu=False, out=None, out_coff=0, g_coff=0, addend=None,
                 scale=None, red=None):
    _chk_s(g, "conv2d_dgrad")
    B, OH, OW, _ = g.shape
    Cgs = pitch(g)
    Cin, KH, KW, Cg = wpack_t.shape
    IH, IW = in_hw
    if out is None:
        out = torch.empty((B, IH, IW, Cin), dtype=g.dtype, device=g.device)
    else:
        _chk_s(out, "conv2d_dgrad out")
        if tuple(out.shape[:3]) != (B, IH, IW) or out.shape[3] < out_coff + Cin or out.dtype != g.dtype:
            raise ValueError(f"conv2d_dgrad: out {tuple(out.shape)} {out.dtype} cannot take a ({B},{IH},{IW},{Cin}) {g.dtype} result at channel {out_coff}")
    if addend is not None:
        _chk_s(addend, "conv2d_dgrad addend")
        if tuple(addend.shape) != (B, IH, IW, Cin) or addend.dtype != g.dtype:
            raise ValueError(f"conv2d_dgrad: addend {tuple(addend.shape)} {addend.dtype} does not match the result")
    lib = _lib.load()
    red_x = red_par = red_out = None
    if red is not None:
        red_x, red_par = red
        _chk_s(red_x, "conv2d_dgrad red_x")
        if tuple(red_x.shape) != (B, IH, IW, Cin) or red_x.dtype != g.dtype:
            raise ValueError(f"conv2d_dgrad: red_x {tuple(red_x.shape)} {red_x.dtype} does not match the result")
        rows = lib.jspsr_conv2d_stats_rows(B, IH, IW)
        red_out = torch.empty((rows, 2, Cin), dtype=torch.float32, device=g.device)
    _lib.check(lib.jspsr_conv2d_dgrad(_dt(g), g.data_ptr(), wpack_t.data_ptr(),
                                      bias.data_ptr() if bias is not None else None, out.data_ptr(),
                                      B, OH, OW, Cg, Cgs, g_coff, IH, IW, Cin, pitch(out), out_coff,
                                      KH, KW, stride, pad, int(relu),
                                      addend.data_ptr() if addend is not None else None,
                                      pitch(addend) if addend is not None else 0,
                                      scale.data_ptr() if scale is not None else None,
                                      red_x.data_ptr() if red is not None else None, pitch(red_x) if red is not None else 0,
                                      red_par.data_ptr() if red is not None else None,
                                      red_out.data_ptr() if red is not None else None, _stream()), "jspsr_conv2d_dgrad")
    return (out, red_out) if red is not None else out


def conv2d_wgrad(G, X, R, C, KH, KW, stride, pad, out=None, accumulate=False, g_coff=0, cg=None, x_coff=0, cx=None,
                 x_affine=None, x_relu=False):
    _chk_s(G, "conv2d_wgrad")
    _chk_s(X, "conv2d_wgrad")
    B, OH, OW, Cg_ = G.shape
    _, IH, IW, Cx_ = X.shape
    Cgs, Cxs = pitch(G), pitch(X)
    cg = Cg_ if cg is None else cg
    cx = Cx_ if cx is None else cx
    if out is None:
        out = torch.empty((R, C, KH, KW), dtype=torch.float32, device=G.device)
    lib = _lib.load()
    dt = _dt(G)
    nbytes = lib.jspsr_conv2d_wgrad_workspace_bytes(dt, B, OH, OW, cg, cx, KH, KW)
    ws = torch.empty(max(nbytes, 16), dtype=torch.uint8, device=G.device)
    _lib.check(lib.jspsr_conv2d_wgrad(dt, G.data_ptr(), cg, Cgs, g_coff, X.data_ptr(), cx, Cxs, x_coff,
                                      out.data_ptr(), R, C, B, OH, OW, IH, IW, KH, KW, stride, pad,
                                      int(accumulate), x_affine.data_ptr() if x_affine is not None else None, int(x_relu),
                                      ws.data_ptr(), _stream()), "jspsr_conv2d_wgrad")
    return out



_ws_cache = {}


def _workspace(dtype_code: int, C: int, nseg: int, device) -> torch.Tensor:
    lib = _lib.load()
    n = lib.jspsr_reduce_workspace_bytes(dtype_code, C, nseg)
    key = (device, _stream())
    buf = _ws_cache.get(key)
    if buf is None or buf.numel() < n:
        buf = torch.empty(max(n, 1 << 20), dtype=torch.uint8, device=device)
        _ws_cache[key] = buf
    return buf


def bn_forward(x, gamma, beta, running_mean, running_var, momentum, eps, training, relu=False, res=None,
               res_scale=1.0, out=None, out_coff=0, partial=None, res_affine=None, stats_only=False):
    _chk_s(x, "bn_forward")
    B, H, W, C = x.shape
    affine = torch.empty((2, C), dtype=torch.float32, device=x.device) if stats_only else None
    if out is None and not stats_only:
        out = torch.empty((B, H, W, C), dtype=x.dtype, device=x.device)
    mean = torch.empty(C, dtype=torch.float32, device=x.device)
    invstd = torch.empty(C, dtype=torch.float32, device=x.device)
    dt = _dt(x)
    ws = _workspace(dt, C, 1, x.device)
    lib = _lib.load()
    _lib.check(lib.jspsr_bn_forward(dt, x.data_ptr(), pitch(x), 0, res.data_ptr() if res is not None else None,
                                    pitch(res) if res is not None else 0, 0, out.data_ptr() if out is not None else None,
                                    pitch(out) if out is not None else 0, out_coff,
                                    gamma.data_ptr(), beta.data_ptr(),
                                    running_mean.data_ptr() if running_mean is not None else None,
                                    running_var.data_ptr() if running_var is not None else None,
                                    float(momentum), float(eps), int(training), int(relu), float(res_scale),
                                    mean.data_ptr(), invstd.data_ptr(), B * H * W, C,
                                    partial.data_ptr() if partial is not None else None,
                                    partial.shape[0] if partial is not None else 0,
                                    res_affine.data_ptr() if res_affine is not None else None,
                                    affine.data_ptr() if affine is not None else None, ws.data_ptr(), _stream()),
               "jspsr_bn_forward")
    return (affine if stats_only else out), mean, invstd


def bn_fold(gamma, beta, running_mean, running_var, eps, res_scale=1.0):
    C = gamma.numel()
    scale = torch.empty(C, dtype=torch.float32, device=gamma.device)
    shift = torch.empty_like(scale)
    _lib.check(_lib.load().jspsr_bn_fold(gamma.data_ptr(), beta.data_ptr(), running_mean.data_ptr(), running_var.data_ptr(),
                                         float(eps), float(res_scale), C, scale.data_ptr(), shift.data_ptr(), _stream()),
               "jspsr_bn_fold")
    return scale, shift


def bn_backward(dy, y, x, gamma, mean, invstd, training, relu, res_scale=1.0, want_dres=False, beta=None,
                grads_into=None, ext_partial=None):
    _chk_s(dy, "bn_backward")
    B, H, W, C = x.shape
    dx = torch.empty((B, H, W, C), dtype=x.dtype, device=x.device)
    dres = torch.empty((B, H, W, C), dtype=x.dtype, device=x.device) if want_dres else None
    if grads_into is not None:
        dgamma, dbeta = grads_into
        for t in (dgamma, dbeta):
            if t.dtype != torch.float32 or not t.is_contiguous() or t.numel() != C or not t.is_cuda:
                raise ValueError("bn_backward: grads_into buffers must be contiguous fp32 of C elements on the GPU")
    else:
        dgamma = torch.empty(C, dtype=torch.float32, device=x.device)
        dbeta = torch.empty(C, dtype=torch.float32, device=x.device)
    dt = _dt(x)
    ws = _workspace(dt, C, 1, x.device)
    lib = _lib.load()
    _lib.check(lib.jspsr_bn_backward(dt, dy.data_ptr(), pitch(dy), 0, y.data_ptr() if y is not None else None,
                                     pitch(y) if y is not None else 0, 0, x.data_ptr(), pitch(x), 0, gamma.data_ptr(),
                                     beta.data_ptr() if beta is not None else None,
                                     mean.data_ptr(), invstd.data_ptr(), int(training), int(relu), float(res_scale),
                                     dx.data_ptr(), dres.data_ptr() if dres is not None else None, dgamma.data_ptr(),
                                     dbeta.data_ptr(), int(grads_into is not None), B * H * W, C, ws.data_ptr(),
                                     ext_partial.data_ptr() if ext_partial is not None else None,
                                     ext_partial.shape[0] if ext_partial is not None else 0,
                                     _stream()), "jspsr_bn_backward")
    if grads_into is not None:
        return dx, dres, None, None
    return dx, dres, dgamma, dbeta


def act_backward(dy, y, relu, want_dz=True, want_dbias=True, dz_channels=None):
    _chk_s(dy, "act_backward")
    B, H, W, C = dy.shape
    dz = None
    if want_dz:
        cz = C if dz_channels is None else dz_channels
        dz = torch.empty((B, H, W, cz), dtype=dy.dtype, device=dy.device) if cz == C else \
            torch.zeros((B, H, W, cz), dtype=dy.dtype, device=dy.device)
    dbias = torch.empty(C, dtype=torch.float32, device=dy.device) if want_dbias else None
    dt = _dt(dy)
    ws = _workspace(dt, C, 1, dy.device)
    lib = _lib.load()
    if y is not None:
        y = nhwc(y)
    _lib.check(lib.jspsr_act_backward(dt, dy.data_ptr(), pitch(dy), 0, y.data_ptr() if y is not None else None,
                                      pitch(y) if y is not None else 0, int(relu),
                                      dz.data_ptr() if dz is not None else None, dz.shape[3] if dz is not None else 0,
                                      dbias.data_ptr() if dbias is not None else None, B * H * W, C, ws.data_ptr(),
                                      _stream()), "jspsr_act_backward")
    return dz, dbias


def gate_pool(x):
    _chk(x, "gate_pool")
    B, H, W, C = x.shape
    avg = torch.empty((B, C), dtype=torch.float32, device=x.device)
    mx = torch.empty_like(avg)
    amax = torch.empty((B, C), dtype=torch.int32, device=x.device)
    dt = _dt(x)
    ws = _workspace(dt, C, B, x.device)
    lib = _lib.load()
    _lib.check(lib.jspsr_gate_pool(dt, x.data_ptr(), B, H * W, C, avg.data_ptr(), mx.data_ptr(), amax.data_ptr(),
                                   ws.data_ptr(), _stream()), "jspsr_gate_pool")
    return avg, mx, amax


def gate_scale(x, s):
    B, H, W, C = x.shape
    y = torch.empty_like(x)
    lib = _lib.load()
    _lib.check(lib.jspsr_gate_scale(_dt(x), x.data_ptr(), s.data_ptr(), y.data_ptr(), B, H * W, C, _stream()),
               "jspsr_gate_scale")
    return y


def gate_backward_reduce(dy, x):
    B, H, W, C = x.shape
    ds = torch.empty((B, C), dtype=torch.float32, device=x.device)
    dt = _dt(x)
    ws = _workspace(dt, C, B, x.device)
    lib = _lib.load()
    _lib.check(lib.jspsr_gate_backward_reduce(dt, dy.data_ptr(), x.data_ptr(), ds.data_ptr(), B, H * W, C,
                                              ws.data_ptr(), _stream()), "jspsr_gate_backward_reduce")
    return ds


def gate_backward_apply(dy, s, davg, dmax, amax):
    B, H, W, C = dy.shape
    dx = torch.empty_like(dy)
    lib = _lib.load()
    _lib.check(lib.jspsr_gate_backward_apply(_dt(dy), dy.data_ptr(), s.data_ptr(), davg.data_ptr(), dmax.data_ptr(),
                                             amax.data_ptr(), dx.data_ptr(), B, H * W, C, _stream()),
               "jspsr_gate_backward_apply")
    return dx


def nchw_to_nhwc(x, dtype, c_pad):
    if x.dtype != torch.float32 or not x.is_contiguous() or not x.is_cuda:
        raise ValueError("nchw_to_nhwc: a contiguous fp32 CUDA tensor (B,C,H,W) is expected")
    B, C, H, W = x.shape
    out = torch.empty((B, H, W, c_pad), dtype=dtype, device=x.device)
    lib = _lib.load()
    _lib.check(lib.jspsr_nchw_to_nhwc(BF16 if dtype == torch.bfloat16 else F32, x.data_ptr(), out.data_ptr(),
                                      B, C, H, W, c_pad, _stream()), "jspsr_nchw_to_nhwc")
    return out


def gate_mlp_forward(avg, mx, w1, w2):
    B, C = avg.shape
    Ch = w1.shape[0]
    s = torch.empty((B, C), dtype=torch.float32, device=avg.device)
    hid = torch.empty((B, 2, Ch), dtype=torch.float32, device=avg.device)
    lib = _lib.load()
    _lib.check(lib.jspsr_gate_mlp_forward(avg.data_ptr(), mx.data_ptr(), w1.data_ptr(), w2.data_ptr(), B, C, Ch, s.data_ptr(),
                                          hid.data_ptr(), _stream()), "jspsr_gate_mlp_forward")
    return s, hid


def gate_mlp_backward(ds, s, hid, avg, mx, w1, w2):
    B, C = avg.shape
    Ch = w1.shape[0]
    davg, dmax = torch.empty_like(avg), torch.empty_like(avg)
    dw1, dw2 = torch.empty_like(w1), torch.empty_like(w2)
    lib = _lib.load()
    ws = torch.empty(lib.jspsr_gate_mlp_backward_workspace_bytes(B, C, Ch) // 4, dtype=torch.float32, device=avg.device)
    _lib.check(lib.jspsr_gate_mlp_backward(ds.data_ptr(), s.data_ptr(), hid.data_ptr(), avg.data_ptr(), mx.data_ptr(), w1.data_ptr(),
                                           w2.data_ptr(), B, C, Ch, davg.data_ptr(), dmax.data_ptr(), dw1.data_ptr(), dw2.data_ptr(),
                                           ws.data_ptr(), _stream()), "jspsr_gate_mlp_backward")
    return davg, dmax, dw1, dw2
```

### jspsr_amd/ops.py

```python
from __future__ import annotations

import collections
import os
import weakref

import torch

from . import _lib
from . import kernels as K


def _stream() -> int:
    return torch.cuda.current_stream().cuda_stream


def _need_gpu(*ts):
    for t in ts:
        if not t.is_cuda:
            raise RuntimeError("jspsr_amd ops run on the GPU only (got a CPU tensor); there is no CPU fallback")
        if t.dtype != torch.float32:
            raise TypeError(f"expected float32, got {t.dtype}")


def prop_forward_raw(dem, weight, offset, w, b, scale, out):
    B, _, H, W = dem.shape
    lib = _lib.load()
    _lib.check(lib.jspsr_prop_forward_f32(dem.data_ptr(), weight.data_ptr(), offset.data_ptr(), offset.shape[1],
                                          w.data_ptr(), b.data_ptr(), float(scale), out.data_ptr(), B, H, W, _stream()),
               "jspsr_prop_forward_f32")


def prop_backward_raw(grad_out, dem, weight, offset, w, gweight, goffset, gw, gb, ws):
    B, _, H, W = dem.shape
    lib = _lib.load()
    _lib.check(lib.jspsr_prop_backward_f32(grad_out.data_ptr(), dem.data_ptr(), weight.data_ptr(), offset.data_ptr(),
                                           offset.shape[1], w.data_ptr(), gweight.data_ptr(), goffset.data_ptr(),
                                           gw.data_ptr() if gw is not None else None,
                                           gb.data_ptr() if gb is not None else None, ws.data_ptr(), B, H, W, _stream()),
               "jspsr_prop_backward_f32")


def prop_backward_fold_raw(ws, B, H, W, gw, gb):
    _lib.check(_lib.load().jspsr_prop_backward_fold_f32(ws.data_ptr(), B, H, W, gw.data_ptr(), gb.data_ptr(), _stream()),
               "jspsr_prop_backward_fold_f32")


def prop_backward_workspace(B, H, W, device):
    n = _lib.load().jspsr_prop_backward_workspace_bytes(B, H, W)
    return torch.empty(max(n, 16), dtype=torch.uint8, device=device)


class _Propagate(torch.autograd.Function):

    @staticmethod
    def forward(ctx, dem, weight, offset, w, b, scale):
        _need_gpu(dem, weight, offset, w, b)
        B, one, H, W = dem.shape
        oc = offset.shape[1]
        if one != 1 or weight.shape != (B, 9, H, W) or offset.shape != (B, oc, H, W) or oc not in (16, 18):
            raise ValueError(f"propagate: bad shapes dem {tuple(dem.shape)} weight {tuple(weight.shape)} offset {tuple(offset.shape)}")
        if w.numel() != 9 or b.numel() != 1:
            raise ValueError("propagate: w must have 9 elements and b 1")
        dem, weight, offset = dem.contiguous(), weight.contiguous(), offset.contiguous()
        w, b = w.contiguous(), b.contiguous()
        out = torch.empty_like(dem)
        lib = _lib.load()
        _lib.check(lib.jspsr_prop_forward_f32(dem.data_ptr(), weight.data_ptr(), offset.data_ptr(), oc,
                                              w.data_ptr(), b.data_ptr(), float(scale), out.data_ptr(),
                                              B, H, W, _stream()), "jspsr_prop_forward_f32")
        ctx.save_for_backward(dem, weight, offset, w)
        return out

    @staticmethod
    def backward(ctx, grad_out):
        dem, weight, offset, w = ctx.saved_tensors
        B, _, H, W = dem.shape
        oc = offset.shape[1]
        grad_out = grad_out.contiguous()
        gweight = torch.empty_like(weight)
        goffset = torch.empty_like(offset)
        gw = torch.empty_like(w)
        gb = torch.empty(1, device=dem.device, dtype=dem.dtype)
        lib = _lib.load()
        ws = torch.empty(lib.jspsr_prop_backward_workspace_bytes(B, H, W), dtype=torch.uint8, device=dem.device)
        _lib.check(lib.jspsr_prop_backward_f32(grad_out.data_ptr(), dem.data_ptr(), weight.data_ptr(),
                                               offset.data_ptr(), oc, w.data_ptr(), gweight.data_ptr(),
                                               goffset.data_ptr(), gw.data_ptr(), gb.data_ptr(), ws.data_ptr(),
                                               B, H, W, _stream()), "jspsr_prop_backward_f32")
        return None, gweight, goffset, gw, gb, None


def propagate(dem, weight, offset, w, b, scale: float = 1.0):
    if dem.requires_grad:
        raise RuntimeError("propagate: dem requires grad, but this operator produces no gradient with respect to the DEM "
                           "(every reference caller detaches it); use propagate_steps for chains that need it")
    return _Propagate.apply(dem, weight, offset, w, b, scale)


def _step_forward(dem, weight, offset, w, b, scale, normalize, out):
    B, _, H, W = dem.shape
    lib = _lib.load()
    _lib.check(lib.jspsr_prop_step_forward_f32(dem.data_ptr(), weight.data_ptr(), offset.data_ptr(), offset.shape[1],
                                               w.data_ptr(), b.data_ptr(), float(scale), int(normalize), out.data_ptr(),
                                               B, H, W, _stream()), "jspsr_prop_step_forward_f32")
    return out


def _step_backward(gout, dem, weight, offset, w, scale, normalize, accumulate, gweight, goffset, gdem, ws):
    B, _, H, W = dem.shape
    lib = _lib.load()
    _lib.check(lib.jspsr_prop_step_backward_f32(gout.data_ptr(), dem.data_ptr(), weight.data_ptr(), offset.data_ptr(),
                                                offset.shape[1], w.data_ptr(), float(scale), int(normalize), int(accumulate),
                                                gweight.data_ptr(), goffset.data_ptr(),
                                                gdem.data_ptr() if gdem is not None else None, None, None, ws.data_ptr(),
                                                B, H, W, _stream()), "jspsr_prop_step_backward_f32")


def _step_workspace(B, H, W, device):
    n = _lib.load().jspsr_prop_step_backward_workspace_bytes(B, H, W)
    return torch.empty(max(n, 16), dtype=torch.uint8, device=device)


class _PropagateSteps(torch.autograd.Function):

    @staticmethod
    def forward(ctx, feat, aff, offset, n_steps, mask_fix, feat_fix):
        _need_gpu(feat, aff, offset)
        B, one, H, W = feat.shape
        oc = offset.shape[1]
        if one != 1 or tuple(aff.shape) != (B, 9, H, W) or tuple(offset.shape) != (B, oc, H, W) or oc not in (16, 18):
            raise ValueError(f"propagate_steps: bad shapes feat {tuple(feat.shape)} aff {tuple(aff.shape)} offset {tuple(offset.shape)}")
        if n_steps < 1:
            raise ValueError("propagate_steps: n_steps must be >= 1")
        aff, offset = aff.contiguous(), offset.contiguous()
        ones = torch.ones(9, device=feat.device)
        zero = torch.zeros(1, device=feat.device)
        cur, inputs, outs = feat.contiguous(), [], []
        for _ in range(n_steps):
            if mask_fix is not None:
                cur = ((1.0 - mask_fix) * cur + mask_fix * feat_fix).contiguous()
            inputs.append(cur)
            cur = _step_forward(cur, aff, offset, ones, zero, 0.0, 0, torch.empty_like(cur))
            outs.append(cur)
        ctx.save_for_backward(aff, offset, ones, mask_fix, *inputs)
        ctx.n = n_steps
        return tuple(outs)

    @staticmethod
    def backward(ctx, *gouts):
        aff, offset, ones, mask_fix = ctx.saved_tensors[:4]
        inputs = ctx.saved_tensors[4:]
        B, _, H, W = inputs[0].shape
        gaff, goff = torch.empty_like(aff), torch.empty_like(offset)
        ws = _step_workspace(B, H, W, aff.device)
        g, gfix = None, None
        first = _PropagateSteps._last(ctx, gouts)
        if first < 0:
            return None, None, None, None, None, None
        for i in range(ctx.n - 1, -1, -1):
            gi = gouts[i]
            if gi is not None:
                g = gi.contiguous() if g is None else g + gi
            if g is None:
                continue
            gin = torch.zeros_like(inputs[i])
            _step_backward(g.contiguous(), inputs[i], aff, offset, ones, 0.0, 0, i != first, gaff, goff, gin, ws)
            if mask_fix is not None:
                gfix = mask_fix * gin if gfix is None else gfix + mask_fix * gin
                gin = (1.0 - mask_fix) * gin
            g = gin
        return g, gaff, goff, None, None, gfix

    @staticmethod
    def _last(ctx, gouts):
        for i in range(ctx.n - 1, -1, -1):
            if gouts[i] is not None:
                return i
        return -1


def propagate_steps(feat, aff, offset, n_steps, mask_fix=None, feat_fix=None):
    if (mask_fix is None) != (feat_fix is None):
        raise ValueError("propagate_steps: mask_fix and feat_fix go together")
    return list(_PropagateSteps.apply(feat, aff, offset, int(n_steps), mask_fix, feat_fix))


class _SampleTaps(torch.autograd.Function):

    @staticmethod
    def forward(ctx, conf, off16, legacy):
        _need_gpu(conf, off16)
        B, _, H, W = conf.shape
        conf = conf.contiguous()
        off = off16.detach().clone().contiguous()
        if not legacy:
            for t in range(8):
                k = t if t < 4 else t + 1
                off[:, 2 * t] -= (k // 3 - 1)
                off[:, 2 * t + 1] -= (k % 3 - 1)
        ones9 = torch.ones(B, 9, H, W, device=conf.device)
        zero = torch.zeros(1, device=conf.device)
        out = torch.empty(8, B, 1, H, W, device=conf.device)
        hots = []
        for t in range(8):
            hot = torch.zeros(9, device=conf.device)
            hot[t if t < 4 else t + 1] = 1.0
            hots.append(hot)
            _step_forward(conf, ones9, off, hot, zero, 0.0, 0, out[t])
        ctx.save_for_backward(conf, off, ones9, *hots)
        return out.permute(1, 0, 2, 3, 4).reshape(B, 8, H, W).contiguous()

    @staticmethod
    def backward(ctx, g):
        conf, off, ones9 = ctx.saved_tensors[:3]
        hots = ctx.saved_tensors[3:]
        B, _, H, W = conf.shape
        gconf = torch.zeros_like(conf)
        scratch_w, scratch_o = torch.empty_like(ones9), torch.empty_like(off)
        ws = _step_workspace(B, H, W, conf.device)
        for t in range(8):
            _step_backward(g[:, t:t + 1].contiguous(), conf, ones9, off, hots[t], 0.0, 0, 0, scratch_w, scratch_o, gconf, ws)
        return gconf, None, None


def sample_taps(conf, off16, legacy=False):
    return _SampleTaps.apply(conf, off16, bool(legacy))


HEAD_CHANNELS = 32


def head_rows():
    rows = []
    for t in range(8):
        k = t if t < 4 else t + 1
        rows += [("w", k), ("o", 2 * t), ("o", 2 * t + 1), ("w", 4) if t == 0 else ("z", 0)]
    return rows


def merge_heads(w_weight, b_weight, w_offset, b_offset):
    nw, no = w_weight.shape[0], w_offset.shape[0]
    base = {"w": 0, "o": nw, "z": nw + no}
    key = (nw, no, w_weight.device)
    idx = _head_index.get(key)
    if idx is None:
        idx = _head_index[key] = torch.tensor([base[kind] + i for kind, i in head_rows()], device=w_weight.device)
    stack_w = torch.cat((w_weight, w_offset, w_weight.new_zeros((1,) + tuple(w_weight.shape[1:]))), 0)
    stack_b = torch.cat((b_weight, b_offset, b_weight.new_zeros(1)), 0)
    return stack_w.index_select(0, idx), stack_b.index_select(0, idx)


_head_index = {}


def split_head(head):
    h = head.reshape(*head.shape[:3], 8, 4)
    logits = torch.cat((h[..., :4, 0], h[..., 0:1, 3], h[..., 4:, 0]), -1)
    return logits, h[..., 1:3].reshape(*head.shape[:3], 16)


class _PropagateHead(torch.autograd.Function):

    @staticmethod
    def forward(ctx, dem, head, w, b, scale):
        _need_gpu(dem, w, b)
        if not head.is_cuda or head.dtype not in (torch.float32, torch.bfloat16):
            raise TypeError("propagate_head: head must be a float32 or bfloat16 GPU tensor")
        B, one, H, W = dem.shape
        if one != 1 or tuple(head.shape) != (B, H, W, HEAD_CHANNELS):
            raise ValueError(f"propagate_head: dem {tuple(dem.shape)} against head {tuple(head.shape)} (want (B,H,W,{HEAD_CHANNELS}))")
        if w.numel() != 9 or b.numel() != 1:
            raise ValueError("propagate_head: w must have 9 elements and b 1")
        dem, head, w, b = dem.contiguous(), head.contiguous(), w.contiguous(), b.contiguous()
        out = torch.empty_like(dem)
        lib = _lib.load()
        _lib.check(lib.jspsr_prop_head_forward(K._dt(head), dem.data_ptr(), head.data_ptr(), w.data_ptr(), b.data_ptr(),
                                               float(scale), out.data_ptr(), B, H, W, _stream()), "jspsr_prop_head_forward")
        ctx.save_for_backward(dem, head, w)
        return out

    @staticmethod
    def backward(ctx, grad_out):
        dem, head, w = ctx.saved_tensors
        B, _, H, W = dem.shape
        grad_out = grad_out.contiguous()
        ghead = torch.empty_like(head)
        gw = torch.empty_like(w)
        gb = torch.empty(1, device=dem.device, dtype=dem.dtype)
        lib = _lib.load()
        ws = torch.empty(max(lib.jspsr_prop_head_backward_workspace_bytes(B, H, W), 16), dtype=torch.uint8, device=dem.device)
        _lib.check(lib.jspsr_prop_head_backward(K._dt(head), grad_out.data_ptr(), dem.data_ptr(), head.data_ptr(),
                                                w.data_ptr(), ghead.data_ptr(), gw.data_ptr(), gb.data_ptr(), ws.data_ptr(),
                                                B, H, W, _stream()), "jspsr_prop_head_backward")
        return None, ghead, gw, gb, None


def propagate_head(dem, head, w, b, scale: float = 1.0):
    if dem.requires_grad:
        raise RuntimeError("propagate_head: dem must be detached (no gradient with respect to the DEM is produced)")
    return _PropagateHead.apply(dem, head, w, b, scale)


HEAD_PLANES = 25


def head_planes_ok(x) -> bool:
    if not x.is_cuda or x.dim() != 4 or x.dtype not in (torch.float32, torch.bfloat16):
        return False
    B, H, W, C = x.shape
    return bool(_lib.load().jspsr_head_ok(K._dt(x), B, H, W, C))


class _HeadPlanes(torch.autograd.Function):

    @staticmethod
    def forward(ctx, x, w25, b25):
        x = K.nhwc(x)
        B, H, W, C = x.shape
        w = w25.detach().reshape(HEAD_PLANES, C).contiguous().float()
        b = b25.detach().contiguous().float()
        planes = torch.empty((B, HEAD_PLANES, H, W), dtype=torch.float32, device=x.device)
        lib = _lib.load()
        _lib.check(lib.jspsr_head_forward(K._dt(x), x.data_ptr(), K.pitch(x), 0, C, w.data_ptr(), b.data_ptr(), planes.data_ptr(),
                                          B, H, W, _stream()), "jspsr_head_forward")
        ctx.save_for_backward(x, w)
        return planes

    @staticmethod
    def backward(ctx, g):
        x, w = ctx.saved_tensors
        B, H, W, C = x.shape
        g = g.contiguous()
        lib = _lib.load()
        dx = torch.empty((B, H, W, C), dtype=x.dtype, device=x.device) if ctx.needs_input_grad[0] else None
        gn = torch.empty((B, H, W, 32), dtype=x.dtype, device=x.device)
        db = torch.empty(HEAD_PLANES, dtype=torch.float32, device=x.device)
        ws = torch.empty(lib.jspsr_head_backward_workspace_bytes(B, H, W), dtype=torch.uint8, device=x.device)
        _lib.check(lib.jspsr_head_backward(K._dt(x), g.data_ptr(), w.data_ptr(), C, dx.data_ptr() if dx is not None else None,
                                           C, 0, gn.data_ptr(), db.data_ptr(), ws.data_ptr(), B, H, W, _stream()),
                   "jspsr_head_backward")
        dW = None
        if ctx.needs_input_grad[1]:
            dW = _wgrad_async(None, gn, x, 32, C, 1, 1, 1, 0)[:HEAD_PLANES]
        return dx, dW, db if ctx.needs_input_grad[2] else None


def head_planes(x, w_weight, b_weight, w_offset, b_offset):
    w25 = torch.cat((w_weight, w_offset), 0)
    b25 = torch.cat((b_weight, b_offset), 0)
    return _HeadPlanes.apply(x, w25, b25)


class _ConvHead1(torch.autograd.Function):

    @staticmethod
    def forward(ctx, x, weight, bias):
        x = K.nhwc(x)
        B, H, W, C = x.shape
        if tuple(weight.shape) != (1, C, 3, 3) or bias is None or bias.numel() != 1:
            raise ValueError(f"conv_head1: weight {tuple(weight.shape)} / bias must be (1,{C},3,3) / (1,)")
        w = weight.detach().contiguous().float()
        b = bias.detach().contiguous().float()
        y = torch.empty((B, 1, H, W), dtype=torch.float32, device=x.device)
        lib = _lib.load()
        _lib.check(lib.jspsr_conv_head1_forward(K._dt(x), x.data_ptr(), K.pitch(x), 0, C, w.data_ptr(), b.data_ptr(),
                                                y.data_ptr(), B, H, W, _stream()), "jspsr_conv_head1_forward")
        ctx.save_for_backward(x, w)
        return y

    @staticmethod
    def backward(ctx, dy):
        x, w = ctx.saved_tensors
        B, H, W, C = x.shape
        dy = dy.contiguous().float()
        lib = _lib.load()
        dx = torch.empty((B, H, W, C), dtype=x.dtype, device=x.device) if ctx.needs_input_grad[0] else None
        dw = torch.empty((1, C, 3, 3), dtype=torch.float32, device=x.device)
        db = torch.empty(1, dtype=torch.float32, device=x.device)
        ws = torch.empty(lib.jspsr_conv_head1_workspace_bytes(B, H, W, C), dtype=torch.uint8, device=x.device)
        _lib.check(lib.jspsr_conv_head1_backward(K._dt(x), dy.data_ptr(), x.data_ptr(), K.pitch(x), 0, C, w.data_ptr(),
                                                 dx.data_ptr() if dx is not None else None, C, 0, dw.data_ptr(),
                                                 db.data_ptr(), ws.data_ptr(), B, H, W, _stream()),
                   "jspsr_conv_head1_backward")
        return dx, dw if ctx.needs_input_grad[1] else None, db if ctx.needs_input_grad[2] else None


def conv_head1(x, weight, bias):
    return _ConvHead1.apply(x, weight, bias)


class _PropagateLogits(torch.autograd.Function):

    @staticmethod
    def forward(ctx, dem, head, w, b, scale):
        _need_gpu(dem, head, w, b)
        B, one, H, W = dem.shape
        if one != 1 or tuple(head.shape) != (B, HEAD_PLANES, H, W) or head.dtype != torch.float32:
            raise ValueError(f"propagate_logits: dem {tuple(dem.shape)} against head {tuple(head.shape)} {head.dtype} (want fp32 (B,{HEAD_PLANES},H,W))")
        if w.numel() != 9 or b.numel() != 1:
            raise ValueError("propagate_logits: w must have 9 elements and b 1")
        dem, head, w, b = dem.contiguous(), head.contiguous(), w.contiguous(), b.contiguous()
        out = torch.empty_like(dem)
        lib = _lib.load()
        _lib.check(lib.jspsr_prop_logits_forward_f32(dem.data_ptr(), head.data_ptr(), w.data_ptr(), b.data_ptr(), float(scale),
                                                     out.data_ptr(), B, H, W, _stream()), "jspsr_prop_logits_forward_f32")
        ctx.save_for_backward(dem, head, w)
        return out

    @staticmethod
    def backward(ctx, grad_out):
        dem, head, w = ctx.saved_tensors
        B, _, H, W = dem.shape
        grad_out = grad_out.contiguous()
        ghead = torch.empty_like(head)
        gw = torch.empty_like(w)
        gb = torch.empty(1, device=dem.device, dtype=dem.dtype)
        lib = _lib.load()
        ws = torch.empty(max(lib.jspsr_prop_backward_workspace_bytes(B, H, W), 16), dtype=torch.uint8, device=dem.device)
        _lib.check(lib.jspsr_prop_logits_backward_f32(grad_out.data_ptr(), dem.data_ptr(), head.data_ptr(), w.data_ptr(),
                                                      ghead.data_ptr(), gw.data_ptr(), gb.data_ptr(), ws.data_ptr(), B, H, W,
                                                      _stream()), "jspsr_prop_logits_backward_f32")
        return None, ghead, gw, gb, None


def propagate_logits(dem, head, w, b, scale: float = 1.0):
    if dem.requires_grad:
        raise RuntimeError("propagate_logits: dem must be detached (no gradient with respect to the DEM is produced)")
    return _PropagateLogits.apply(dem, head, w, b, scale)




_weights_epoch = 0


def invalidate_packed_weights():
    global _weights_epoch
    _weights_epoch += 1


repack_after_step = os.environ.get("JSPSR_REPACK_ALL", "0") != "0"
_pack_registry = {}
_pack_table = None


def _packed(param, w, mode, c_pad, dtype):
    if not isinstance(param, torch.nn.Parameter):
        return K.pack_weight(w, mode, c_pad, dtype)
    cache = param.__dict__.setdefault("_jspsr_packs", {})
    key = (mode, c_pad, dtype, w.data_ptr())
    hit = cache.get(key)
    stamp = (param._version, _weights_epoch)
    if hit is not None and hit[1] == stamp:
        return hit[0]
    if len(cache) > 8:
        cache.clear()
    packed = K.pack_weight(w, mode, c_pad, dtype)
    cache[key] = (packed, stamp)
    if id(param) not in _pack_registry:
        _pack_registry[id(param)] = weakref.ref(param, lambda _, k=id(param): _pack_registry.pop(k, None))
    return packed


def repack_all():
    global _pack_table
    import numpy as np
    entries = []
    for ref in list(_pack_registry.values()):
        p = ref()
        if p is None or not p.is_cuda:
            continue
        for (mode, c_pad, dtype, ptr), (packed, _) in p.__dict__.get("_jspsr_packs", {}).items():
            if ptr == p.data_ptr() and p.dim() == 4 and p.is_contiguous():
                entries.append((p, mode, c_pad, dtype, packed))
    if not entries:
        return 0
    sig = tuple((p.data_ptr(), packed.data_ptr(), mode, c_pad) for p, mode, c_pad, _, packed in entries)
    if _pack_table is None or _pack_table[0] != sig:
        desc = np.zeros(len(entries), dtype=np.dtype([("w", "<u8"), ("out", "<u8"), ("start", "<i8"), ("total", "<i8"),
                                                      ("O", "<i4"), ("I", "<i4"), ("KH", "<i4"), ("KW", "<i4"), ("mode", "<i4"),
                                                      ("c_pad", "<i4"), ("dtype", "<i4"), ("reserved", "<i4")]))
        start, chunk = 0, _lib.load().jspsr_pack_chunk()
        for i, (p, mode, c_pad, dtype, packed) in enumerate(entries):
            O, I, KH, KW = p.shape
            total = packed.numel()
            desc[i] = (p.data_ptr(), packed.data_ptr(), start, total, O, I, KH, KW, mode, c_pad, K._dt(packed), 0)
            start += (total + chunk - 1) // chunk
        table = torch.from_numpy(desc.view(np.uint8).copy()).to(entries[0][0].device)
        _pack_table = (sig, table, start)
    _, table, grand = _pack_table
    _lib.check(_lib.load().jspsr_pack_weights_multi(table.data_ptr(), len(entries), grand, _stream()), "jspsr_pack_weights_multi")
    for p, mode, c_pad, dtype, packed in entries:
        p.__dict__["_jspsr_packs"][(mode, c_pad, dtype, p.data_ptr())] = (packed, (p._version, _weights_epoch))
    return len(entries)


def pad_channels(x: torch.Tensor, mult: int) -> torch.Tensor:
    c = x.shape[-1]
    p = (-c) % mult
    return x if p == 0 else torch.nn.functional.pad(x, (0, p))


def _wgrad_into(param, G, X, R, C, KH, KW, stride, pad, **kw):
    gbuf = param.grad if param is not None and getattr(param, "_jspsr_direct_grad", False) else None
    if (gbuf is not None and gbuf.dtype == torch.float32 and gbuf.is_contiguous() and gbuf.is_cuda
            and tuple(gbuf.shape) == (R, C, KH, KW)):
        K.conv2d_wgrad(G, X, R, C, KH, KW, stride, pad, out=gbuf, accumulate=True, **kw)
        ready = getattr(param, "_jspsr_grad_ready", None)
        if ready is not None:
            ready(param)
        return None
    return K.conv2d_wgrad(G, X, R, C, KH, KW, stride, pad, **kw)


_aux_streams = {}
_marks = {}
RUN_AHEAD = int(os.environ.get("JSPSR_RUN_AHEAD", "16"))
wgrad_async = os.environ.get("JSPSR_WGRAD_ASYNC", "1") != "0"
wgrad_after_dgrad = os.environ.get("JSPSR_WGRAD_AFTER_DGRAD", "0") != "0"
wgrad_one_stream = os.environ.get("JSPSR_WGRAD_ONE_STREAM", "0") != "0"
bn_reduce_fused = os.environ.get("JSPSR_BN_REDUCE_FUSE", "1") != "0"


def aux_streams():
    return list(_aux_streams.values())


def _wgrad_async(param, G, X, R, C, KH, KW, stride, pad, **kw):
    if not wgrad_async:
        return _wgrad_into(param, G, X, R, C, KH, KW, stride, pad, **kw)
    cur = torch.cuda.current_stream()
    key = 0 if wgrad_one_stream else cur.cuda_stream
    aux = _aux_streams.get(key)
    if aux is None:
        aux = _aux_streams[key] = torch.cuda.Stream(device=G.device)
    aux.wait_stream(cur)
    with torch.cuda.stream(aux):
        dW = _wgrad_into(param, G, X, R, C, KH, KW, stride, pad, **kw)
    for t_ in kw.values():
        if isinstance(t_, torch.Tensor):
            t_.record_stream(aux)
    G.record_stream(aux)
    X.record_stream(aux)
    if not torch.cuda.is_current_stream_capturing():
        marks = _marks.setdefault(cur.cuda_stream, collections.deque())
        marks.append(cur.record_event())
        if len(marks) > RUN_AHEAD:
            marks.popleft().synchronize()
    if dW is not None:
        cur.wait_stream(aux)
        dW.record_stream(cur)
    return dW


def _bn_sink(gparam, bparam):
    bufs = []
    for p_ in (gparam, bparam):
        g_ = p_.grad if p_ is not None and getattr(p_, "_jspsr_direct_grad", False) else None
        if g_ is None or g_.dtype != torch.float32 or not g_.is_contiguous() or not g_.is_cuda or g_.dim() != 1:
            return None
        bufs.append(g_)
    return tuple(bufs)


def _bn_ready(gparam, bparam):
    for p_ in (gparam, bparam):
        ready = getattr(p_, "_jspsr_grad_ready", None)
        if ready is not None:
            ready(p_)


class SliceBuffer:

    def __init__(self, B, H, W, C, dtype, device):
        self.buf = torch.empty((B, H, W, C), dtype=dtype, device=device)
        self.deferred = None
        self.deferred_event = None
        self.deposit_events = []
        self.expected_deposits = 0
        self.pending_deposits = 0

    def take_deferred(self):
        g, self.deferred = self.deferred, None
        if g is not None:
            if len(self.deposit_events) != self.pending_deposits:
                raise RuntimeError(f"SliceBuffer: {len(self.deposit_events)} of {self.pending_deposits} deposits into the parked "
                                   "gradient had run when it was taken (autograd order changed?)")
            cur = torch.cuda.current_stream()
            for ev in self.deposit_events:
                cur.wait_event(ev)
            self.deposit_events = []
        return g

    def slice(self, lo, n, shape=None):
        if lo < 0 or lo + n > self.buf.shape[3]:
            raise ValueError(f"SliceBuffer: channels [{lo}, {lo + n}) outside a {self.buf.shape[3]}-channel buffer")
        if shape is not None and tuple(shape) != tuple(self.buf.shape[:3]):
            raise ValueError(f"SliceBuffer: producer shape {tuple(shape)} != buffer {tuple(self.buf.shape[:3])}")
        v = self.buf.narrow(3, lo, n).detach()
        if not (v.is_contiguous() or K.is_slice(v)):
            raise ValueError("SliceBuffer: slice start / buffer width must be a multiple of 16 bytes")
        return v

    def join(self, parts, lo=0, defer=0):
        return _Join.apply(self, lo, defer, *parts)


class _Join(torch.autograd.Function):
    @staticmethod
    def forward(ctx, holder, lo, defer, *parts):
        ctx.holder, ctx.defer = holder, int(defer)
        ctx.widths = [p.shape[3] for p in parts]
        n = sum(ctx.widths)
        for p, w in zip(parts, ctx.widths):
            if p.untyped_storage().data_ptr() != holder.buf.untyped_storage().data_ptr():
                raise RuntimeError("SliceBuffer.join: a part does not live in this buffer")
        return holder.buf.narrow(3, lo, n).detach()

    @staticmethod
    def backward(ctx, g):
        outs, off = [], 0
        keep = len(ctx.widths) - ctx.defer
        for i, w in enumerate(ctx.widths):
            outs.append(g.narrow(3, off, w) if i < keep else None)
            if i == keep:
                ctx.holder.deferred = g.narrow(3, off, sum(ctx.widths[keep:]))
                ctx.holder.deferred_event = torch.cuda.current_stream().record_event()
                ctx.holder.deposit_events = []
                ctx.holder.pending_deposits = ctx.holder.expected_deposits
            off += w
        return (None, None, None) + tuple(outs)


class _Conv(torch.autograd.Function):

    @staticmethod
    def forward(ctx, x, weight, bias, stride, pad, relu, transposed, want_stats=False, dest=None):
        x = K.nhwc(x)
        cdt = x.dtype
        e = K.epc(cdt)
        B, H, W, Cp = x.shape
        if Cp % e:
            raise ValueError(f"conv: input channels {Cp} must be padded to a multiple of {e} (ops.pad_channels)")
        w = weight.detach().contiguous()
        ctx.wparam = weight if isinstance(weight, torch.nn.Parameter) else None
        bias_d = bias.detach().contiguous() if bias is not None else None
        if not transposed:
            O, I, KH, KW = w.shape
            if Cp < I:
                raise ValueError("conv: input has fewer channels than the weight")
            out = None
            if dest is not None:
                out = dest[0].slice(dest[1], O, (B, (H + 2 * pad - KH) // stride + 1, (W + 2 * pad - KW) // stride + 1))
            y = K.conv2d_forward(x, _packed(weight, w, 0, Cp, cdt), bias_d, stride, pad, relu, stats=want_stats, out=out)
            if want_stats:
                y, st = y
                ctx.cfg = (stride, pad, relu, transposed, bias is not None)
                ctx.save_for_backward(x, w, None)
                ctx.mark_non_differentiable(st)
                return y, st
        else:
            I, O, KH, KW = w.shape
            if Cp != I or stride != 2 or pad != 1 or KH != 3:
                raise ValueError("conv_transpose: only k3 s2 p1 op1 without channel padding is built")
            if dest is not None:
                raise ValueError("conv_transpose: dest is not supported")
            y = K.conv2d_dgrad(x, _packed(weight, w, 1, Cp, cdt), (2 * H, 2 * W), 2, 1, bias=bias_d, relu=relu)
        ctx.cfg = (stride, pad, relu, transposed, bias is not None)
        ctx.save_for_backward(x, w, y if relu else None)
        return y

    @staticmethod
    def backward(ctx, dy, *unused):
        stride, pad, relu, transposed, has_bias = ctx.cfg
        x, w, y = ctx.saved_tensors
        cdt = x.dtype
        e = K.epc(cdt)
        dy = K.nhwc(dy)
        Co = dy.shape[3]
        Cg = (Co + e - 1) // e * e
        dbias = None
        if Co % e == 0 and (relu or has_bias):
            dz, dbias = K.act_backward(dy, y, relu, want_dz=relu, want_dbias=has_bias)
            if dz is None:
                dz = dy
        else:
            dz = pad_channels(dy * (y > 0) if relu else dy, e).contiguous()
            if has_bias:
                dbias = K.act_backward(dz, None, False, want_dz=False, want_dbias=True)[1][:Co]
        B, H, W, Cp = x.shape
        dx = dW = None
        if not transposed:
            O, I, KH, KW = w.shape
            if ctx.needs_input_grad[0]:
                if Cp != I:
                    raise RuntimeError("conv backward: gradient w.r.t. a channel-padded input is not supported")
                dx = K.conv2d_dgrad(dz, _packed(ctx.wparam, w, 1, Cg, cdt), (H, W), stride, pad)
            if ctx.needs_input_grad[1]:
                dW = _wgrad_async(ctx.wparam, dz, x, O, I, KH, KW, stride, pad)
        else:
            I, O, KH, KW = w.shape
            if ctx.needs_input_grad[0]:
                dx = K.conv2d_forward(dz, _packed(ctx.wparam, w, 0, Cg, cdt), None, 2, 1, False)
            if ctx.needs_input_grad[1]:
                dW = _wgrad_async(ctx.wparam, x, dz, I, O, KH, KW, 2, 1)
        return dx, dW, dbias, None, None, None, None, None, None


def conv2d(x, weight, bias=None, stride=1, pad=0, relu=False, dest=None):
    return _Conv.apply(x, weight, bias, stride, pad, relu, False, False, dest)


def conv2d_with_stats(x, weight, stride=1, pad=0):
    return _Conv.apply(x, weight, None, stride, pad, False, False, True)


def conv_transpose2d(x, weight):
    return _Conv.apply(x, weight, None, 2, 1, False, True)


class _BatchNorm(torch.autograd.Function):

    @staticmethod
    def forward(ctx, x, gamma, beta, running_mean, running_var, momentum, eps, training, relu, res, res_scale,
                partial=None, dest=None):
        x = K.nhwc(x)
        res_c = K.nhwc(res) if res is not None else None
        rs = float(res_scale) if res is not None else 1.0
        out = dest[0].slice(dest[1], x.shape[3], x.shape[:3]) if dest is not None else None
        y, mean, invstd = K.bn_forward(x, gamma.detach(), beta.detach(), running_mean, running_var, momentum, eps,
                                       training, relu, res_c, rs, partial=partial if training else None, out=out)
        mode = 0 if not relu else (1 if res is not None else 2)
        ctx.gb = tuple(p if isinstance(p, torch.nn.Parameter) else None for p in (gamma, beta))
        ctx.cfg = (training, mode, rs, res is not None)
        ctx.save_for_backward(x, y if mode == 1 else None, gamma.detach(), beta.detach(), mean, invstd)
        return y

    @staticmethod
    def backward(ctx, dy):
        training, relu, rs, has_res = ctx.cfg
        x, y, gamma, beta, mean, invstd = ctx.saved_tensors
        sink = _bn_sink(*ctx.gb)
        dx, dres, dgamma, dbeta = K.bn_backward(K.nhwc(dy), y, x, gamma, mean, invstd, training, relu, rs,
                                                want_dres=has_res and ctx.needs_input_grad[9], beta=beta, grads_into=sink)
        if sink is not None:
            _bn_ready(*ctx.gb)
        if has_res and ctx.needs_input_grad[9] and dres is None:
            dres = dy
        return dx, dgamma, dbeta, None, None, None, None, None, None, dres, None, None, None


def batch_norm(x, gamma, beta, running_mean, running_var, momentum, eps, training, relu=False, res=None, res_scale=1.0,
               partial=None, dest=None):
    return _BatchNorm.apply(x, gamma, beta, running_mean, running_var, momentum, eps, training, relu, res, res_scale,
                            partial, dest)


fold_shortcut_bn = os.environ.get("JSPSR_BN_FOLD_SHORTCUT", "1") != "0"
fuse_bn1_input = os.environ.get("JSPSR_FUSE_BN1", "1") != "0"


class _ResUnit(torch.autograd.Function):

    @staticmethod
    def forward(ctx, x, w1, g1, b1, w2, g2, b2, wd, gd, bd, stride, scale, act, bns, dest, grad_extra=None):
        ctx.grad_extra = grad_extra
        x = K.nhwc(x)
        cdt, e = x.dtype, K.epc(x.dtype)
        B, H, W, Cp = x.shape
        O, I = w1.shape[:2]
        if Cp != I or Cp % e or O % e:
            raise ValueError(f"res_unit: {Cp} input channels against weight {tuple(w1.shape)} (multiples of {e} needed)")
        has_d = wd is not None
        (rm1, rv1, mom1, eps1, tr1), (rm2, rv2, mom2, eps2, tr2) = bns[0], bns[1]
        w1d, w2d = w1.detach().contiguous(), w2.detach().contiguous()
        g1d, b1d, g2d, b2d = g1.detach(), b1.detach(), g2.detach(), b2.detach()

        def conv_bn(inp, wt, k, st, pad, gam, bet, rm, rv, mom, eps, tr, relu, res=None, rs=1.0, out=None, par=None,
                    res_affine=None, stats_only=False, in_affine=None):
            z = K.conv2d_forward(inp, _packed(par, wt, 0, inp.shape[3], cdt), None, st, pad, False, stats=tr,
                                 in_affine=in_affine, in_relu=in_affine is not None)
            z, part = z if tr else (z, None)
            y, mean, invstd = K.bn_forward(z, gam, bet, rm, rv, mom, eps, tr, relu, res, rs, partial=part, out=out,
                                           res_affine=res_affine, stats_only=stats_only)
            return z, y, mean, invstd

        OH1, OW1 = (H + 2 - 3) // stride + 1, (W + 2 - 3) // stride + 1
        fuse1 = fuse_bn1_input and K.fused_input_ok(cdt, B, OH1, OW1, O, O, 3, 3, 1, 1)
        if fuse1:
            z1, aff1, m1, i1 = conv_bn(x, w1d, 3, stride, 1, g1d, b1d, rm1, rv1, mom1, eps1, tr1, True, par=w1, stats_only=True)
            y1 = None
        else:
            z1, y1, m1, i1 = conv_bn(x, w1d, 3, stride, 1, g1d, b1d, rm1, rv1, mom1, eps1, tr1, True, par=w1)
            aff1 = None
        if has_d:
            rmd, rvd, momd, epsd, trd = bns[2]
            wdd, gdd, bdd = wd.detach().contiguous(), gd.detach(), bd.detach()
            if fold_shortcut_bn:
                zd, r_aff, md, idd = conv_bn(x, wdd, 1, stride, 0, gdd, bdd, rmd, rvd, momd, epsd, trd, False, par=wd, stats_only=True)
                r = zd
            else:
                zd, r, md, idd = conv_bn(x, wdd, 1, stride, 0, gdd, bdd, rmd, rvd, momd, epsd, trd, False, par=wd)
                r_aff = None
        else:
            r_aff = None
            if stride != 1 or O != I:
                raise ValueError("res_unit: identity shortcut needs stride 1 and equal channel counts")
            wdd = gdd = bdd = zd = md = idd = None
            trd = False
            r = x
        out_v = dest[0].slice(dest[1], O, z1.shape[:3]) if dest is not None else None
        z2, out, m2, i2 = conv_bn(z1 if fuse1 else y1, w2d, 3, 1, 1, g2d, b2d, rm2, rv2, mom2, eps2, tr2, bool(act), r, float(scale),
                                  out_v, par=w2, res_affine=r_aff, in_affine=aff1)
        ctx.cfg = (stride, float(scale), bool(act), has_d, tr1, tr2, trd)
        ctx.wparams = tuple(p if isinstance(p, torch.nn.Parameter) else None for p in (w1, w2, wd))
        ctx.bparams = tuple(p if isinstance(p, torch.nn.Parameter) else None for p in (g1, b1, g2, b2, gd, bd))
        ctx.save_for_backward(x, w1d, g1d, b1d, z1, m1, i1, y1, w2d, g2d, b2d, z2, m2, i2, out if act else None,
                              wdd, gdd, bdd, zd, md, idd, aff1)
        return out

    @staticmethod
    def backward(ctx, dout):
        stride, scale, act, has_d, tr1, tr2, trd = ctx.cfg
        (x, w1, g1, b1, z1, m1, i1, y1, w2, g2, b2, z2, m2, i2, out, wd, gd, bd, zd, md, idd, aff1) = ctx.saved_tensors
        cdt = x.dtype
        B, H, W, Cin = x.shape
        O = w1.shape[0]
        dout = K.nhwc(dout)
        need_x = ctx.needs_input_grad[0]
        pg1, pb1, pg2, pb2, pgd, pbd = ctx.bparams
        sink2, sink1 = _bn_sink(pg2, pb2), _bn_sink(pg1, pb1)
        dz2, dres, dg2, db2 = K.bn_backward(dout, out, z2, g2, m2, i2, tr2, 1 if act else 0, scale,
                                            want_dres=(need_x or has_d), beta=b2, grads_into=sink2)
        if sink2 is not None:
            _bn_ready(pg2, pb2)
        if dres is None:
            dres = dout
        p1, p2, pd = ctx.wparams

        def wgrad2():
            if aff1 is not None:
                return _wgrad_async(p2, dz2, z1, O, O, 3, 3, 1, 1, x_affine=aff1, x_relu=True)
            return _wgrad_async(p2, dz2, y1, O, O, 3, 3, 1, 1)

        if not wgrad_after_dgrad:
            dW2 = wgrad2()
        Bz, Hz, Wz, _ = z1.shape
        part1 = None
        if bn_reduce_fused and tr1 and K.dgrad_reduce_ok(cdt, Bz, Hz, Wz, O, O, 3, 3, 1, 1) and z1.is_contiguous():
            par1 = K.bn_reduce_params(g1, b1, m1, i1)
            dy1, part1 = K.conv2d_dgrad(dz2, _packed(p2, w2, 1, O, cdt), z1.shape[1:3], 1, 1, red=(z1, par1))
        else:
            dy1 = K.conv2d_dgrad(dz2, _packed(p2, w2, 1, O, cdt), z1.shape[1:3], 1, 1)
        if wgrad_after_dgrad:
            dW2 = wgrad2()
        del dz2
        dz1, _, dg1, db1 = K.bn_backward(dy1, None, z1, g1, m1, i1, tr1, 2, 1.0, beta=b1, grads_into=sink1, ext_partial=part1)
        if sink1 is not None:
            _bn_ready(pg1, pb1)
        del dy1
        dW1 = None if wgrad_after_dgrad else _wgrad_async(p1, dz1, x, O, Cin, 3, 3, stride, 1)
        dWd = dgd = dbd = None
        side = dres
        deposit = None
        if isinstance(ctx.grad_extra, tuple):
            holder, off, n = ctx.grad_extra
            if holder.deferred is not None and has_d and need_x:
                cur = torch.cuda.current_stream()
                cur.wait_event(holder.deferred_event)
                deposit = holder.deferred.narrow(3, off, n)
                if tuple(deposit.shape) != tuple(x.shape):
                    raise RuntimeError(f"res_unit: parked gradient slice {tuple(deposit.shape)} does not match the input {tuple(x.shape)}")
                if deposit.dtype != x.dtype or not (deposit.is_contiguous() or K.is_slice(deposit)):
                    holder.pending_deposits -= 1
                    deposit = None
                else:
                    deposit.record_stream(cur)
            elif holder.deferred is not None:
                holder.pending_deposits -= 1
        extra = ctx.grad_extra.take_deferred() if (ctx.grad_extra is not None and not isinstance(ctx.grad_extra, tuple)) else deposit
        if extra is not None:
            extra = K.nhwc(extra)
            if tuple(extra.shape) != tuple(x.shape):
                raise RuntimeError(f"res_unit: deferred gradient {tuple(extra.shape)} does not match the input {tuple(x.shape)}")
            if not (has_d and need_x):
                side, extra = side + extra, None
        if has_d:
            sinkd = _bn_sink(pgd, pbd)
            dzd, _, dgd, dbd = K.bn_backward(dres, None, zd, gd, md, idd, trd, 0, 1.0, beta=bd, grads_into=sinkd)
            if sinkd is not None:
                _bn_ready(pgd, pbd)
            dWd = _wgrad_async(pd, dzd, x, O, Cin, 1, 1, stride, 0)
            side = K.conv2d_dgrad(dzd, _packed(pd, wd, 1, O, cdt), (H, W), stride, 0, addend=extra) if need_x else None
        dx = None
        if need_x and deposit is not None:
            K.conv2d_dgrad(dz1, _packed(p1, w1, 1, O, cdt), (H, W), stride, 1, addend=K.nhwc(side), out=deposit)
            ctx.grad_extra[0].deposit_events.append(torch.cuda.current_stream().record_event())
        elif need_x:
            dx = K.conv2d_dgrad(dz1, _packed(p1, w1, 1, O, cdt), (H, W), stride, 1, addend=K.nhwc(side))
        if wgrad_after_dgrad:
            dW1 = _wgrad_async(p1, dz1, x, O, Cin, 3, 3, stride, 1)
        return (dx, dW1, dg1, db1, dW2, dg2, db2, dWd, dgd, dbd, None, None, None, None, None, None)


def conv_bn_infer(x, weight, gamma, beta, bn, stride, pad, relu=False, res=None, res_scale=1.0, dest=None):
    x = K.nhwc(x)
    rm, rv, _, eps, training = bn
    if training or rm is None:
        raise RuntimeError("conv_bn_infer: BatchNorm must be in eval mode with running statistics")
    sc, sh = K.bn_fold(gamma.detach(), beta.detach(), rm, rv, eps, res_scale if res is not None else 1.0)
    O, I, KH, KW = weight.shape
    B, H, W, Cp = x.shape
    out = None
    if dest is not None:
        out = dest[0].slice(dest[1], O, (B, (H + 2 * pad - KH) // stride + 1, (W + 2 * pad - KW) // stride + 1))
    return K.conv2d_forward(x, _packed(weight, weight.detach().contiguous(), 0, Cp, x.dtype), sh, stride, pad, relu, out=out,
                            scale=sc, addend=K.nhwc(res) if res is not None else None)


def conv_transpose_bn_infer(x, weight, gamma, beta, bn, relu=True, dest=None):
    x = K.nhwc(x)
    rm, rv, _, eps, training = bn
    if training or rm is None:
        raise RuntimeError("conv_transpose_bn_infer: BatchNorm must be in eval mode with running statistics")
    I, O, KH, KW = weight.shape
    B, H, W, Cp = x.shape
    if Cp != I or KH != 3:
        raise ValueError("conv_transpose: only k3 s2 p1 op1 without channel padding is built")
    sc, sh = K.bn_fold(gamma.detach(), beta.detach(), rm, rv, eps, 1.0)
    out = dest[0].slice(dest[1], O, (B, 2 * H, 2 * W)) if dest is not None else None
    return K.conv2d_dgrad(x, _packed(weight, weight.detach().contiguous(), 1, Cp, x.dtype), (2 * H, 2 * W), 2, 1, bias=sh,
                          relu=relu, out=out, scale=sc)


def res_unit_infer(x, w1, g1, b1, w2, g2, b2, wd, gd, bd, stride, scale, act, bns, dest=None):
    y1 = conv_bn_infer(x, w1, g1, b1, bns[0], stride, 1, relu=True)
    r = conv_bn_infer(x, wd, gd, bd, bns[2], stride, 0) if wd is not None else x
    return conv_bn_infer(y1, w2, g2, b2, bns[1], 1, 1, relu=bool(act), res=r, res_scale=scale, dest=dest)


def res_unit(x, w1, g1, b1, w2, g2, b2, wd, gd, bd, stride, scale, act, bns, dest=None, grad_extra=None):
    if not torch.is_grad_enabled() and not any(b[4] for b in bns):
        return res_unit_infer(x, w1, g1, b1, w2, g2, b2, wd, gd, bd, stride, scale, act, bns, dest)
    return _ResUnit.apply(x, w1, g1, b1, w2, g2, b2, wd, gd, bd, stride, scale, act, bns, dest, grad_extra)


def _gate_mlp(avg, mx, w1, w2):
    f = torch.nn.functional
    h = lambda v: f.linear(f.relu(f.linear(v, w1.flatten(1))), w2.flatten(1))
    return torch.sigmoid(h(avg) + h(mx))


class _ChannelGate(torch.autograd.Function):

    @staticmethod
    def forward(ctx, x, w1, w2):
        x = x.contiguous()
        avg, mx, amax = K.gate_pool(x)
        w1f, w2f = w1.detach().float().flatten(1).contiguous(), w2.detach().float().flatten(1).contiguous()
        s, hid = K.gate_mlp_forward(avg, mx, w1f, w2f)
        y = K.gate_scale(x, s)
        ctx.save_for_backward(x, avg, mx, amax, s, hid, w1f, w2f)
        ctx.wshapes = (w1.shape, w2.shape, w1.dtype, w2.dtype)
        return y

    @staticmethod
    def backward(ctx, dy):
        x, avg, mx, amax, s, hid, w1f, w2f = ctx.saved_tensors
        dy = dy.contiguous()
        ds = K.gate_backward_reduce(dy, x)
        davg, dmax, dw1, dw2 = K.gate_mlp_backward(ds, s, hid, avg, mx, w1f, w2f)
        dx = K.gate_backward_apply(dy, s, davg, dmax, amax)
        s1, s2, t1, t2 = ctx.wshapes
        return dx, dw1.reshape(s1).to(t1), dw2.reshape(s2).to(t2)


def channel_gate(x, w1, w2):
    return _ChannelGate.apply(x, w1, w2)
```

Before: 34.74 Mpixel/s.

## Save packed ReLU bit mask in BN forward instead of full output for backward

```diff
diff --git a/include/jspsr_hip.h b/include/jspsr_hip.h
--- a/include/jspsr_hip.h
+++ b/include/jspsr_hip.h
@@ -132,12 +132,13 @@
 
 size_t jspsr_reduce_workspace_bytes(int dtype, int C, int nseg);
 
+size_t jspsr_bn_mask_bytes(int dtype, long long npix, int C);
 int jspsr_bn_forward(int dtype, const void* x, int x_cs, int x_coff, const void* res, int r_cs, int r_coff,
                      void* y, int y_cs, int y_coff, const float* gamma, const float* beta,
                      float* running_mean, float* running_var, float momentum, float eps, int training,
                      int relu, float res_scale, float* save_mean, float* save_invstd, long long npix, int C,
                      const float* ext_partial, int ext_rows, const float* res_affine, float* affine_out,
-                     void* workspace, jspsr_stream_t stream);
+                     void* mask_out, void* workspace, jspsr_stream_t stream);
 
 int jspsr_bn_fold(const float* gamma, const float* beta, const float* running_mean, const float* running_var,
                   float eps, float res_scale, int C, float* scale, float* shift, jspsr_stream_t stream);
@@ -148,7 +149,7 @@
                       const void* x, int x_cs, int x_coff, const float* gamma, const float* beta, const float* save_mean,
                       const float* save_invstd, int training, int relu, float res_scale, void* dx, void* dres,
                       float* dgamma, float* dbeta, int accumulate, long long npix, int C, void* workspace,
-                      const float* ext_partial, int ext_rows, jspsr_stream_t stream);
+                      const float* ext_partial, int ext_rows, const void* mask, jspsr_stream_t stream);
 
 int jspsr_act_backward(int dtype, const void* dy, int dy_cs, int dy_coff, const void* y, int y_cs, int relu, void* dz,
                        int dz_cs, float* dbias, long long npix, int C, void* workspace, jspsr_stream_t stream);
diff --git a/jspsr_amd/_lib.py b/jspsr_amd/_lib.py
--- a/jspsr_amd/_lib.py
+++ b/jspsr_amd/_lib.py
@@ -8,7 +8,7 @@
 _HERE = os.path.dirname(os.path.abspath(__file__))
 SO_PATH = os.environ.get("JSPSR_LAB_LIB") or os.path.join(_HERE, "lib", "libjspsr_hip.so")
 CSRC = os.path.join(_HERE, "csrc")
-ABI_VERSION = 20
+ABI_VERSION = 21
 
 _lock = threading.Lock()
 _lib = None
@@ -56,10 +56,11 @@
     "jspsr_conv2d_wgrad": (c_i, [c_i, c_p, c_i, c_i, c_i, c_p, c_i, c_i, c_i, c_p] + [c_i] * 12 + [c_p, c_i, c_p, c_p]),
     "jspsr_reduce_workspace_bytes": (ctypes.c_size_t, [c_i, c_i, c_i]),
     "jspsr_bn_forward": (c_i, [c_i, c_p, c_i, c_i, c_p, c_i, c_i, c_p, c_i, c_i, c_p, c_p, c_p, c_p, c_f, c_f, c_i,
-                               c_i, c_f, c_p, c_p, c_ll, c_i, c_p, c_i, c_p, c_p, c_p, c_p]),
+                               c_i, c_f, c_p, c_p, c_ll, c_i, c_p, c_i, c_p, c_p, c_p, c_p, c_p]),
+    "jspsr_bn_mask_bytes": (ctypes.c_size_t, [c_i, c_ll, c_i]),
     "jspsr_bn_reduce_params": (c_i, [c_p, c_p, c_p, c_p, c_i, c_p, c_p]),
     "jspsr_bn_backward": (c_i, [c_i, c_p, c_i, c_i, c_p, c_i, c_i, c_p, c_i, c_i, c_p, c_p, c_p, c_p, c_i, c_i, c_f,
-                                c_p, c_p, c_p, c_p, c_i, c_ll, c_i, c_p, c_p, c_i, c_p]),
+                                c_p, c_p, c_p, c_p, c_i, c_ll, c_i, c_p, c_p, c_i, c_p, c_p]),
     "jspsr_act_backward": (c_i, [c_i, c_p, c_i, c_i, c_p, c_i, c_i, c_p, c_i, c_p, c_ll, c_i, c_p, c_p]),
     "jspsr_gate_pool": (c_i, [c_i, c_p, c_i, c_ll, c_i, c_p, c_p, c_p, c_p, c_p]),
     "jspsr_gate_scale": (c_i, [c_i, c_p, c_p, c_p, c_i, c_ll, c_i, c_p]),
diff --git a/jspsr_amd/csrc/common.hip b/jspsr_amd/csrc/common.hip
--- a/jspsr_amd/csrc/common.hip
+++ b/jspsr_amd/csrc/common.hip
@@ -51,7 +51,7 @@
 int conv_dynq_override() { return g_conv_dynq.load(std::memory_order_relaxed); }
 }
 
-extern "C" int jspsr_abi_version(void) { return 20; }
+extern "C" int jspsr_abi_version(void) { return 21; }
 extern "C" int jspsr_conv_dynamic_queue(int on) { return jspsr::g_conv_dynq.exchange(on < 0 ? -1 : (on ? 1 : 0), std::memory_order_relaxed); }
 extern "C" long long jspsr_launch_count(const char* what) {
   if (!what) return -1;
diff --git a/jspsr_amd/csrc/elementwise.hip b/jspsr_amd/csrc/elementwise.hip
--- a/jspsr_amd/csrc/elementwise.hip
+++ b/jspsr_amd/csrc/elementwise.hip
@@ -37,7 +37,7 @@
 }
 
 template <typename T>
-__device__ __forceinline__ void store_vec(T* p, const float (&f)[V<T>::N]) {
+__device__ __forceinline__ uint4 pack_vec(const float (&f)[V<T>::N]) {
   uint4 raw;
   if constexpr (sizeof(T) == 4) {
     raw.x = __float_as_uint(f[0]); raw.y = __float_as_uint(f[1]); raw.z = __float_as_uint(f[2]); raw.w = __float_as_uint(f[3]);
@@ -47,7 +47,19 @@
     raw.z = bf16_bits(f[4]) | (bf16_bits(f[5]) << 16);
     raw.w = bf16_bits(f[6]) | (bf16_bits(f[7]) << 16);
   }
-  *reinterpret_cast<uint4*>(p) = raw;
+  return raw;
+}
+template <typename T>
+__device__ __forceinline__ void store_vec(T* p, const float (&f)[V<T>::N]) { *reinterpret_cast<uint4*>(p) = pack_vec<T>(f); }
+
+template <typename T>
+__device__ __forceinline__ unsigned char relu_bits(const uint4& raw) {
+  float f[V<T>::N];
+  unpack<T>(raw, f);
+  unsigned m = 0;
+#pragma unroll
+  for (int k = 0; k < V<T>::N; ++k) m |= (f[k] > 0.f ? 1u : 0u) << k;
+  return (unsigned char)m;
 }
 
 struct Slice {
@@ -222,6 +234,17 @@
 }
 
 template <typename T>
+__device__ __forceinline__ uint4 keep_bits(const uint4& raw, unsigned m) {
+  unsigned w[4] = {raw.x, raw.y, raw.z, raw.w};
+#pragma unroll
+  for (int j = 0; j < 4; ++j) {
+    if constexpr (sizeof(T) == 4) w[j] &= 0u - ((m >> j) & 1u);
+    else w[j] &= ((0u - ((m >> (2 * j)) & 1u)) & 0xffffu) | ((0u - ((m >> (2 * j + 1)) & 1u)) & 0xffff0000u);
+  }
+  return make_uint4(w[0], w[1], w[2], w[3]);
+}
+
+template <typename T>
 __global__ __launch_bounds__(TX * TY) void bn_stats_kernel(const T* __restrict__ x, int cs, int coff, RedGeom g,
                                                           float* __restrict__ partial) {
   constexpr int N = V<T>::N;
@@ -298,13 +321,15 @@
   shift[c] = (beta[c] - mean[c] * sc) * res_scale;
 }
 
-template <typename T, bool RES>
+template <typename T, bool RES, bool MASK>
 __global__ __launch_bounds__(TX * TY) void bn_apply_kernel(const T* __restrict__ x, int x_cs, int x_coff,
                                                           const T* __restrict__ res, int r_cs, int r_coff,
                                                           T* __restrict__ y, int y_cs, int y_coff,
                                                           const float* __restrict__ scale, const float* __restrict__ shift,
-                                                          const float* __restrict__ raff, float res_scale, int relu, RedGeom g) {
+                                                          const float* __restrict__ raff, float res_scale, int relu,
+                                                          unsigned char* __restrict__ mask, RedGeom g) {
   constexpr int N = V<T>::N;
+  const int groups = g.C / N;
   float sc[N], sh[N], rsc[N], rsh[N];
   const int c0 = lane_map<N>(g).c;
   if (c0 < g.C) { load_param<N>(scale + c0, sc); load_param<N>(shift + c0, sh); }
@@ -327,20 +352,25 @@
           if (relu) v = fmaxf(v, 0.f);
           f[k] = v;
         }
-        store_vec<T>(y + (size_t)pix * y_cs + y_coff + c, f);
+        const uint4 o = pack_vec<T>(f);
+        *reinterpret_cast<uint4*>(y + (size_t)pix * y_cs + y_coff + c) = o;
+        if constexpr (MASK) mask[(size_t)pix * groups + c / N] = relu_bits<T>(o);
       });
 }
 
-template <typename T, int RELU>
+template <typename T, int RELU, bool DRES>
 __global__ __launch_bounds__(TX * TY) void bn_bwd_reduce_kernel(const T* __restrict__ dy, int dy_cs, int dy_coff,
                                                                const T* __restrict__ y, int y_cs, int y_coff,
                                                                const T* __restrict__ x, int x_cs, int x_coff,
                                                                const float* __restrict__ mean,
                                                                const float* __restrict__ invstd,
                                                                const float* __restrict__ gamma,
-                                                               const float* __restrict__ beta, RedGeom g,
+                                                               const float* __restrict__ beta,
+                                                               const unsigned char* __restrict__ mask,
+                                                               T* __restrict__ dres, RedGeom g,
                                                                float* __restrict__ partial) {
-  constexpr int N = V<T>::N, NTEN = RELU == 1 ? 3 : 2;
+  constexpr int N = V<T>::N, NTEN = (RELU == 1 || RELU == 3) ? 3 : 2;
+  const int groups = g.C / N;
   float mu[N], is[N], ga[N], be[N];
   const int c0 = lane_map<N>(g).c;
   if (c0 < g.C) {
@@ -353,16 +383,22 @@
         raw[0] = load_raw<T>(dy + (size_t)pix * dy_cs + dy_coff + c);
         raw[1] = load_raw<T>(x + (size_t)pix * x_cs + x_coff + c);
         if constexpr (RELU == 1) raw[2] = load_raw<T>(y + (size_t)pix * y_cs + y_coff + c);
+        if constexpr (RELU == 3) raw[2].x = mask[(size_t)pix * groups + c / N];
       },
-      [&](long long, int, const uint4 (&raw)[NTEN], float (&acc)[2][N]) {
+      [&](long long pix, int c, const uint4 (&raw)[NTEN], float (&acc)[2][N]) {
         float d[N], xv[N], yv[N];
+        unsigned m = 0;
+        if constexpr (RELU == 3) m = raw[2].x;
+        if constexpr (RELU == 1 && DRES) m = relu_bits<T>(raw[2]);
+        if constexpr (DRES) *reinterpret_cast<uint4*>(dres + (size_t)pix * g.C + c) = keep_bits<T>(raw[0], m);
         unpack<T>(raw[0], d);
         unpack<T>(raw[1], xv);
-        if constexpr (RELU == 1) unpack<T>(raw[2], yv);
+        if constexpr (RELU == 1 && !DRES) unpack<T>(raw[2], yv);
 #pragma unroll
         for (int i = 0; i < N; ++i) {
           const float xhat = (xv[i] - mu[i]) * is[i];
-          const bool off = RELU == 1 ? !(yv[i] > 0.f) : (RELU == 2 ? !(ga[i] * xhat + be[i] > 0.f) : false);
+          const bool off = (RELU == 3 || (RELU == 1 && DRES)) ? !((m >> i) & 1u)
+                           : (RELU == 1 ? !(yv[i] > 0.f) : (RELU == 2 ? !(ga[i] * xhat + be[i] > 0.f) : false));
           const float dz = off ? 0.f : d[i];
           acc[0][i] += dz;
           acc[1][i] += dz * xhat;
@@ -394,9 +430,10 @@
                                                               const float* __restrict__ mean, const float* __restrict__ invstd,
                                                               const float* __restrict__ gamma, const float* __restrict__ beta,
                                                               const float* __restrict__ coef,
+                                                              const unsigned char* __restrict__ mask,
                                                               T* __restrict__ dx, T* __restrict__ dres, RedGeom g) {
-  constexpr int N = V<T>::N, NTEN = RELU == 1 ? 3 : 2;
-  const int C = g.C;
+  constexpr int N = V<T>::N, NTEN = (RELU == 1 || RELU == 3) ? 3 : 2;
+  const int C = g.C, groups = C / N;
   float mu[N], is[N], k0[N], ka[N], kb[N], ga[N], be[N];
   const int c0 = lane_map<N>(g).c;
   if (c0 < C) {
@@ -410,6 +447,7 @@
         raw[0] = load_raw<T>(dy + (size_t)pix * dy_cs + dy_coff + c);
         raw[1] = load_raw<T>(x + (size_t)pix * x_cs + x_coff + c);
         if constexpr (RELU == 1) raw[2] = load_raw<T>(y + (size_t)pix * y_cs + y_coff + c);
+        if constexpr (RELU == 3) raw[2].x = mask[(size_t)pix * groups + c / N];
       },
       [&](long long, long long pix, int c, const uint4 (&raw)[NTEN]) {
         float d[N], xv[N], yv[N], o[N];
@@ -419,7 +457,8 @@
 #pragma unroll
         for (int k = 0; k < N; ++k) {
           const float xhat = (xv[k] - mu[k]) * is[k];
-          const bool off = RELU == 1 ? !(yv[k] > 0.f) : (RELU == 2 ? !(ga[k] * xhat + be[k] > 0.f) : false);
+          const bool off = RELU == 1 ? !(yv[k] > 0.f)
+                                     : (RELU == 2 ? !(ga[k] * xhat + be[k] > 0.f) : (RELU == 3 ? !((raw[2].x >> k) & 1u) : false));
           const float dz = off ? 0.f : d[k];
           d[k] = dz;
           o[k] = k0[k] * (dz - ka[k] - xhat * kb[k]);
@@ -668,11 +707,12 @@
                                 float* running_mean, float* running_var, float momentum, float eps, int training,
                                 int relu, float res_scale, float* save_mean, float* save_invstd, long long npix, int C,
                                 const float* ext_partial, int ext_rows, const float* res_affine, float* affine_out,
-                                void* workspace, jspsr_stream_t stream) {
+                                void* mask_out, void* workspace, jspsr_stream_t stream) {
   if (int e = check_c(dtype, C, "bn_forward")) return e;
   if (!x || (!y && !affine_out) || !gamma || !beta || !save_mean || !save_invstd || !workspace || npix <= 0)
     return fail(JSPSR_EINVAL, "bn_forward: null pointer or empty tensor");
   if (res_affine && !res) return fail(JSPSR_EINVAL, "bn_forward: res_affine without a residual operand");
+  if (mask_out && (!res || !relu || !y)) return fail(JSPSR_EINVAL, "bn_forward: mask_out needs an output with residual and ReLU");
   if (!training && (!running_mean || !running_var)) return fail(JSPSR_EINVAL, "bn_forward: eval mode needs running stats");
   const int vec = dtype == JSPSR_F32 ? 4 : 8;
   if (x_cs % vec || x_coff % vec || y_cs % vec || y_coff % vec || (res && (r_cs % vec || r_coff % vec)))
@@ -704,10 +744,11 @@
   if (int e = check_launch("bn_finalize")) return e;
   if (!y) return JSPSR_OK;
   const RedGeom ga = make_red(npix, 1, C, vec);
-#define BN_APPLY(R) DISPATCH(dtype, hipLaunchKernelGGL((bn_apply_kernel<T, R>), red_grid(ga, vec), dim3(TX, TY), 0, s,             \
+#define BN_APPLY(R, M) DISPATCH(dtype, hipLaunchKernelGGL((bn_apply_kernel<T, R, M>), red_grid(ga, vec), dim3(TX, TY), 0, s,       \
                                      static_cast<const T*>(x), x_cs, x_coff, static_cast<const T*>(res), r_cs, r_coff,        \
-                                     static_cast<T*>(y), y_cs, y_coff, scale, shift, res_affine, res_scale, relu, ga))
-  if (res) { BN_APPLY(true); } else { BN_APPLY(false); }
+                                     static_cast<T*>(y), y_cs, y_coff, scale, shift, res_affine, res_scale, relu,             \
+                                     static_cast<unsigned char*>(mask_out), ga))
+  if (mask_out) { BN_APPLY(true, true); } else if (res) { BN_APPLY(true, false); } else { BN_APPLY(false, false); }
 #undef BN_APPLY
   return check_launch("bn_apply");
 }
@@ -723,6 +764,12 @@
   par[3 * C + c] = -mean[c] * invstd[c];
 }
 
+extern "C" size_t jspsr_bn_mask_bytes(int dtype, long long npix, int C) {
+  const int vec = dtype == JSPSR_F32 ? 4 : 8;
+  if (npix <= 0 || C <= 0 || C % vec) return 0;
+  return (size_t)npix * (size_t)(C / vec);
+}
+
 extern "C" int jspsr_bn_reduce_params(const float* gamma, const float* beta, const float* save_mean, const float* save_invstd, int C,
                                       float* par, jspsr_stream_t stream) {
   if (!gamma || !beta || !save_mean || !save_invstd || !par || C <= 0) return fail(JSPSR_EINVAL, "bn_reduce_params: bad arguments");
@@ -735,22 +782,26 @@
                                  const void* x, int x_cs, int x_coff, const float* gamma, const float* beta, const float* save_mean,
                                  const float* save_invstd, int training, int relu, float res_scale, void* dx, void* dres,
                                  float* dgamma, float* dbeta, int accumulate, long long npix, int C, void* workspace,
-                                 const float* ext_partial, int ext_rows, jspsr_stream_t stream) {
+                                 const float* ext_partial, int ext_rows, const void* mask, jspsr_stream_t stream) {
   if (int e = check_c(dtype, C, "bn_backward")) return e;
   if (!dy || !x || !gamma || !save_mean || !save_invstd || !dx || !dgamma || !dbeta || !workspace || npix <= 0 ||
-      (relu == 1 && !y) || (relu == 2 && !beta) || relu < 0 || relu > 2)
+      (relu == 1 && !y && !mask) || (relu == 2 && !beta) || relu < 0 || relu > 2)
     return fail(JSPSR_EINVAL, "bn_backward: null pointer, empty tensor or bad relu mode");
   const int vec = dtype == JSPSR_F32 ? 4 : 8;
-  if (dy_cs % vec || dy_coff % vec || x_cs % vec || x_coff % vec || (relu == 1 && (y_cs % vec || y_coff % vec)))
+  if (dy_cs % vec || dy_coff % vec || x_cs % vec || x_coff % vec || (relu == 1 && !mask && (y_cs % vec || y_coff % vec)))
     return fail(JSPSR_EINVAL, "bn_backward: channel pitches/offsets must be multiples of %d", vec);
   hipStream_t s = static_cast<hipStream_t>(stream);
   float* ws = static_cast<float*>(workspace);
   float* coef = ws;
   float* partial = ws + 3 * C;
   const RedGeom g = make_red(npix, 1, C, vec);
-#define BN_BWD_REDUCE(R) DISPATCH(dtype, hipLaunchKernelGGL((bn_bwd_reduce_kernel<T, R>), red_grid(g, vec), dim3(TX, TY), 0, s, \
+  const unsigned char* mk = relu == 1 ? static_cast<const unsigned char*>(mask) : nullptr;
+  const int mode = (relu == 1 && mk) ? 3 : relu;
+  const bool premask = relu == 1 && dres && !ext_partial;
+#define BN_BWD_REDUCE(R, D) DISPATCH(dtype, hipLaunchKernelGGL((bn_bwd_reduce_kernel<T, R, D>), red_grid(g, vec), dim3(TX, TY), 0, s, \
                                      static_cast<const T*>(dy), dy_cs, dy_coff, static_cast<const T*>(y), y_cs, y_coff,     \
-                                     static_cast<const T*>(x), x_cs, x_coff, save_mean, save_invstd, gamma, beta, g, partial))
+                                     static_cast<const T*>(x), x_cs, x_coff, save_mean, save_invstd, gamma, beta, mk,        \
+                                     static_cast<T*>(dres), g, partial))
   int rows = g.chunks;
   if (ext_partial) {
     if (ext_rows <= 0) return fail(JSPSR_EINVAL, "bn_backward: ext_rows must be positive");
@@ -763,18 +814,25 @@
       rows = ext_rows;
     }
   } else {
-    if (relu == 0) { BN_BWD_REDUCE(0); } else if (relu == 1) { BN_BWD_REDUCE(1); } else { BN_BWD_REDUCE(2); }
+    if (mode == 0) { BN_BWD_REDUCE(0, false); }
+    else if (mode == 2) { BN_BWD_REDUCE(2, false); }
+    else if (mode == 1) { if (premask) { BN_BWD_REDUCE(1, true); } else { BN_BWD_REDUCE(1, false); } }
+    else { if (premask) { BN_BWD_REDUCE(3, true); } else { BN_BWD_REDUCE(3, false); } }
     if (int e = check_launch("bn_bwd_reduce")) return e;
   }
 #undef BN_BWD_REDUCE
   hipLaunchKernelGGL(bn_bwd_finalize_kernel, dim3((C + 3) / 4), dim3(256), 0, s, partial, rows, C, npix, gamma,
                      save_invstd, training, res_scale, accumulate, dgamma, dbeta, coef);
   if (int e = check_launch("bn_bwd_finalize")) return e;
-#define BN_BWD_APPLY(R) DISPATCH(dtype, hipLaunchKernelGGL((bn_bwd_apply_kernel<T, R>), red_grid(g, vec), dim3(TX, TY), 0, s,  \
-                                     static_cast<const T*>(dy), dy_cs, dy_coff, static_cast<const T*>(y), y_cs, y_coff,     \
-                                     static_cast<const T*>(x), x_cs, x_coff, save_mean, save_invstd, gamma, beta, coef,     \
-                                     static_cast<T*>(dx), static_cast<T*>(dres), g))
-  if (relu == 0) { BN_BWD_APPLY(0); } else if (relu == 1) { BN_BWD_APPLY(1); } else { BN_BWD_APPLY(2); }
+#define BN_BWD_APPLY(R, DY, CS, OFF, DRES) DISPATCH(dtype, hipLaunchKernelGGL((bn_bwd_apply_kernel<T, R>), red_grid(g, vec), dim3(TX, TY), 0, s, \
+                                     static_cast<const T*>(DY), CS, OFF, static_cast<const T*>(y), y_cs, y_coff,            \
+                                     static_cast<const T*>(x), x_cs, x_coff, save_mean, save_invstd, gamma, beta, coef, mk, \
+                                     static_cast<T*>(dx), static_cast<T*>(DRES), g))
+  if (premask) { BN_BWD_APPLY(0, dres, C, 0, nullptr); }
+  else if (mode == 0) { BN_BWD_APPLY(0, dy, dy_cs, dy_coff, dres); }
+  else if (mode == 1) { BN_BWD_APPLY(1, dy, dy_cs, dy_coff, dres); }
+  else if (mode == 2) { BN_BWD_APPLY(2, dy, dy_cs, dy_coff, dres); }
+  else { BN_BWD_APPLY(3, dy, dy_cs, dy_coff, dres); }
 #undef BN_BWD_APPLY
   return check_launch("bn_bwd_apply");
 }
diff --git a/jspsr_amd/kernels.py b/jspsr_amd/kernels.py
--- a/jspsr_amd/kernels.py
+++ b/jspsr_amd/kernels.py
@@ -195,7 +195,7 @@
 
 
 def bn_forward(x, gamma, beta, running_mean, running_var, momentum, eps, training, relu=False, res=None,
-               res_scale=1.0, out=None, out_coff=0, partial=None, res_affine=None, stats_only=False):
+               res_scale=1.0, out=None, out_coff=0, partial=None, res_affine=None, stats_only=False, want_mask=False):
     _chk_s(x, "bn_forward")
     B, H, W, C = x.shape
     affine = torch.empty((2, C), dtype=torch.float32, device=x.device) if stats_only else None
@@ -206,6 +206,7 @@
     dt = _dt(x)
     ws = _workspace(dt, C, 1, x.device)
     lib = _lib.load()
+    mask = torch.empty(lib.jspsr_bn_mask_bytes(dt, B * H * W, C), dtype=torch.uint8, device=x.device) if want_mask else None
     _lib.check(lib.jspsr_bn_forward(dt, x.data_ptr(), pitch(x), 0, res.data_ptr() if res is not None else None,
                                     pitch(res) if res is not None else 0, 0, out.data_ptr() if out is not None else None,
                                     pitch(out) if out is not None else 0, out_coff,
@@ -217,8 +218,11 @@
                                     partial.data_ptr() if partial is not None else None,
                                     partial.shape[0] if partial is not None else 0,
                                     res_affine.data_ptr() if res_affine is not None else None,
-                                    affine.data_ptr() if affine is not None else None, ws.data_ptr(), _stream()),
+                                    affine.data_ptr() if affine is not None else None,
+                                    mask.data_ptr() if mask is not None else None, ws.data_ptr(), _stream()),
                "jspsr_bn_forward")
+    if want_mask:
+        return (affine if stats_only else out), mean, invstd, mask
     return (affine if stats_only else out), mean, invstd
 
 
@@ -233,7 +237,7 @@
 
 
 def bn_backward(dy, y, x, gamma, mean, invstd, training, relu, res_scale=1.0, want_dres=False, beta=None,
-                grads_into=None, ext_partial=None):
+                grads_into=None, ext_partial=None, mask=None):
     _chk_s(dy, "bn_backward")
     B, H, W, C = x.shape
     dx = torch.empty((B, H, W, C), dtype=x.dtype, device=x.device)
@@ -249,6 +253,9 @@
     dt = _dt(x)
     ws = _workspace(dt, C, 1, x.device)
     lib = _lib.load()
+    if mask is not None and (mask.dtype != torch.uint8 or not mask.is_contiguous() or
+                             mask.numel() != lib.jspsr_bn_mask_bytes(dt, B * H * W, C)):
+        raise ValueError("bn_backward: mask is not the bit mask bn_forward(want_mask=True) made for this shape")
     _lib.check(lib.jspsr_bn_backward(dt, dy.data_ptr(), pitch(dy), 0, y.data_ptr() if y is not None else None,
                                      pitch(y) if y is not None else 0, 0, x.data_ptr(), pitch(x), 0, gamma.data_ptr(),
                                      beta.data_ptr() if beta is not None else None,
@@ -257,7 +264,7 @@
                                      dbeta.data_ptr(), int(grads_into is not None), B * H * W, C, ws.data_ptr(),
                                      ext_partial.data_ptr() if ext_partial is not None else None,
                                      ext_partial.shape[0] if ext_partial is not None else 0,
-                                     _stream()), "jspsr_bn_backward")
+                                     mask.data_ptr() if mask is not None else None, _stream()), "jspsr_bn_backward")
     if grads_into is not None:
         return dx, dres, None, None
     return dx, dres, dgamma, dbeta
diff --git a/jspsr_amd/ops.py b/jspsr_amd/ops.py
--- a/jspsr_amd/ops.py
+++ b/jspsr_amd/ops.py
@@ -520,6 +520,7 @@
 wgrad_after_dgrad = os.environ.get("JSPSR_WGRAD_AFTER_DGRAD", "0") != "0"
 wgrad_one_stream = os.environ.get("JSPSR_WGRAD_ONE_STREAM", "0") != "0"
 bn_reduce_fused = os.environ.get("JSPSR_BN_REDUCE_FUSE", "1") != "0"
+bn_relu_mask = os.environ.get("JSPSR_BN_RELU_MASK", "1") != "0"
 
 
 def aux_streams():
@@ -728,21 +729,25 @@
         res_c = K.nhwc(res) if res is not None else None
         rs = float(res_scale) if res is not None else 1.0
         out = dest[0].slice(dest[1], x.shape[3], x.shape[:3]) if dest is not None else None
-        y, mean, invstd = K.bn_forward(x, gamma.detach(), beta.detach(), running_mean, running_var, momentum, eps,
-                                       training, relu, res_c, rs, partial=partial if training else None, out=out)
         mode = 0 if not relu else (1 if res is not None else 2)
+        masked = mode == 1 and bn_relu_mask
+        y, mean, invstd, *mk = K.bn_forward(x, gamma.detach(), beta.detach(), running_mean, running_var, momentum, eps,
+                                            training, relu, res_c, rs, partial=partial if training else None, out=out,
+                                            want_mask=masked)
         ctx.gb = tuple(p if isinstance(p, torch.nn.Parameter) else None for p in (gamma, beta))
         ctx.cfg = (training, mode, rs, res is not None)
-        ctx.save_for_backward(x, y if mode == 1 else None, gamma.detach(), beta.detach(), mean, invstd)
+        ctx.save_for_backward(x, y if mode == 1 and not masked else None, gamma.detach(), beta.detach(), mean, invstd,
+                              mk[0] if masked else None)
         return y
 
     @staticmethod
     def backward(ctx, dy):
         training, relu, rs, has_res = ctx.cfg
-        x, y, gamma, beta, mean, invstd = ctx.saved_tensors
+        x, y, gamma, beta, mean, invstd, mask = ctx.saved_tensors
         sink = _bn_sink(*ctx.gb)
         dx, dres, dgamma, dbeta = K.bn_backward(K.nhwc(dy), y, x, gamma, mean, invstd, training, relu, rs,
-                                                want_dres=has_res and ctx.needs_input_grad[9], beta=beta, grads_into=sink)
+                                                want_dres=has_res and ctx.needs_input_grad[9], beta=beta, grads_into=sink,
+                                                mask=mask)
         if sink is not None:
             _bn_ready(*ctx.gb)
         if has_res and ctx.needs_input_grad[9] and dres is None:
@@ -777,13 +782,13 @@
         g1d, b1d, g2d, b2d = g1.detach(), b1.detach(), g2.detach(), b2.detach()
 
         def conv_bn(inp, wt, k, st, pad, gam, bet, rm, rv, mom, eps, tr, relu, res=None, rs=1.0, out=None, par=None,
-                    res_affine=None, stats_only=False, in_affine=None):
+                    res_affine=None, stats_only=False, in_affine=None, want_mask=False):
             z = K.conv2d_forward(inp, _packed(par, wt, 0, inp.shape[3], cdt), None, st, pad, False, stats=tr,
                                  in_affine=in_affine, in_relu=in_affine is not None)
             z, part = z if tr else (z, None)
-            y, mean, invstd = K.bn_forward(z, gam, bet, rm, rv, mom, eps, tr, relu, res, rs, partial=part, out=out,
-                                           res_affine=res_affine, stats_only=stats_only)
-            return z, y, mean, invstd
+            y, mean, invstd, *mk = K.bn_forward(z, gam, bet, rm, rv, mom, eps, tr, relu, res, rs, partial=part, out=out,
+                                                res_affine=res_affine, stats_only=stats_only, want_mask=want_mask)
+            return (z, y, mean, invstd, mk[0]) if want_mask else (z, y, mean, invstd)
 
         OH1, OW1 = (H + 2 - 3) // stride + 1, (W + 2 - 3) // stride + 1
         fuse1 = fuse_bn1_input and K.fused_input_ok(cdt, B, OH1, OW1, O, O, 3, 3, 1, 1)
@@ -810,19 +815,20 @@
             trd = False
             r = x
         out_v = dest[0].slice(dest[1], O, z1.shape[:3]) if dest is not None else None
-        z2, out, m2, i2 = conv_bn(z1 if fuse1 else y1, w2d, 3, 1, 1, g2d, b2d, rm2, rv2, mom2, eps2, tr2, bool(act), r, float(scale),
-                                  out_v, par=w2, res_affine=r_aff, in_affine=aff1)
+        masked = bool(act) and bn_relu_mask
+        z2, out, m2, i2, *mk2 = conv_bn(z1 if fuse1 else y1, w2d, 3, 1, 1, g2d, b2d, rm2, rv2, mom2, eps2, tr2, bool(act), r, float(scale),
+                                        out_v, par=w2, res_affine=r_aff, in_affine=aff1, want_mask=masked)
         ctx.cfg = (stride, float(scale), bool(act), has_d, tr1, tr2, trd)
         ctx.wparams = tuple(p if isinstance(p, torch.nn.Parameter) else None for p in (w1, w2, wd))
         ctx.bparams = tuple(p if isinstance(p, torch.nn.Parameter) else None for p in (g1, b1, g2, b2, gd, bd))
-        ctx.save_for_backward(x, w1d, g1d, b1d, z1, m1, i1, y1, w2d, g2d, b2d, z2, m2, i2, out if act else None,
-                              wdd, gdd, bdd, zd, md, idd, aff1)
+        ctx.save_for_backward(x, w1d, g1d, b1d, z1, m1, i1, y1, w2d, g2d, b2d, z2, m2, i2, out if act and not masked else None,
+                              wdd, gdd, bdd, zd, md, idd, aff1, mk2[0] if masked else None)
         return out
 
     @staticmethod
     def backward(ctx, dout):
         stride, scale, act, has_d, tr1, tr2, trd = ctx.cfg
-        (x, w1, g1, b1, z1, m1, i1, y1, w2, g2, b2, z2, m2, i2, out, wd, gd, bd, zd, md, idd, aff1) = ctx.saved_tensors
+        (x, w1, g1, b1, z1, m1, i1, y1, w2, g2, b2, z2, m2, i2, out, wd, gd, bd, zd, md, idd, aff1, mask2) = ctx.saved_tensors
         cdt = x.dtype
         B, H, W, Cin = x.shape
         O = w1.shape[0]
@@ -831,7 +837,7 @@
         pg1, pb1, pg2, pb2, pgd, pbd = ctx.bparams
         sink2, sink1 = _bn_sink(pg2, pb2), _bn_sink(pg1, pb1)
         dz2, dres, dg2, db2 = K.bn_backward(dout, out, z2, g2, m2, i2, tr2, 1 if act else 0, scale,
-                                            want_dres=(need_x or has_d), beta=b2, grads_into=sink2)
+                                            want_dres=(need_x or has_d), beta=b2, grads_into=sink2, mask=mask2)
         if sink2 is not None:
             _bn_ready(pg2, pb2)
         if dres is None:
```

Result: faster. 35.31 Mpixel/s (median of 6 runs) (+1.6%).
